# kubeai-project/kubeai

Hardware: AMD Instinct MI355X
Metric: output_tokens_per_s (k6 multi-turn chat) (higher is better)
Workload: dtype fp8; 1 GPU; model=llama-3-8b, global_batch=40, seq_len=8192, parallelism=dp1, prefix_cache=True

## Files before the change

### kubeai_amd/csrc/attention_decode.hip

```cpp
#include <torch/extension.h>

#include <type_traits>

#include "common.h"

namespace {

constexpr int kWaves = 2;
constexpr int kBlockThreads = kWaves * WAVE_SIZE;
constexpr int kBS = 16;
typedef __attribute__((ext_vector_type(2))) __bf16 bf16x2v;
constexpr int kPad = 8;

template <int G, typename CT = ushort, int HD = 128, bool CAP = false>
__launch_bounds__(kBlockThreads) __global__ void paged_decode_kernel(
    ushort* __restrict__ out,
    const ushort* __restrict__ q,
    const CT* __restrict__ k_cache,
    const CT* __restrict__ v_cache,
    const int32_t* __restrict__ block_tables,
    const int32_t* __restrict__ seq_lens,
    const float scale, const float softcap, const int window,
    const int n_kv, const int max_blocks,
    const int64_t q_stride, const int n_splits,
    float* __restrict__ part_o,
    float* __restrict__ part_ml) {
  const int b = blockIdx.x / (n_kv * n_splits);
  const int rem = blockIdx.x % (n_kv * n_splits);
  const int kh = rem / n_splits;
  const int split = rem % n_splits;
  const int n_q = n_kv * G;
  const int wave = threadIdx.x / WAVE_SIZE;
  const int lane = threadIdx.x % WAVE_SIZE;
  const int L = seq_lens[b];
  const int n_blocks = (L + kBS - 1) / kBS;
  const int w0 = (window > 0) ? max(0, L - window) : 0;
  const int blk_base = w0 / kBS;
  const int n_eff = n_blocks - blk_base;
  const int chunk = (n_eff + n_splits - 1) / n_splits;
  const int blk_lo = blk_base + split * chunk;
  const int blk_hi = min(n_blocks, blk_lo + chunk);

  constexpr int PARTS = HD / 32;
  constexpr int TOKP = 64 / PARTS;
  constexpr int EPL = HD / 64;
  __shared__ CT k_lds[kWaves][2][kBS][HD + kPad];
  __shared__ CT v_lds[kWaves][2][kBS][HD + kPad];
  __shared__ float merge_o[kWaves][G][HD];
  __shared__ float merge_ml[kWaves][G][2];

  const int tok_of = lane / PARTS;
  const int part = lane % PARTS;

  uint32_t q_pack[G][16];
#pragma unroll
  for (int g = 0; g < G; ++g) {
    const uint32_t* qp = reinterpret_cast<const uint32_t*>(
        q + (int64_t)b * q_stride + (int64_t)(kh * G + g) * HD + part * 32);
#pragma unroll
    for (int i = 0; i < 16; ++i) q_pack[g][i] = qp[i];
  }

  float m[G], l[G], o[G][EPL];
#pragma unroll
  for (int g = 0; g < G; ++g) {
    m[g] = -INFINITY;
    l[g] = 0.f;
#pragma unroll
    for (int e = 0; e < EPL; ++e) o[g][e] = 0.f;
  }

  const int32_t* bt = block_tables + (int64_t)b * max_blocks;

  using StageVec = std::conditional_t<sizeof(CT) == 2, ushort8, uint64_t>;
  constexpr int NS = (kBS * HD / 8) / WAVE_SIZE;
  StageVec stage_k[NS], stage_v[NS];

  auto issue_loads = [&](int blk_i) {
    const int64_t blk = bt[blk_i];
    const CT* base_k = k_cache + ((blk * n_kv + kh) * kBS) * HD;
    const CT* base_v = v_cache + ((blk * n_kv + kh) * kBS) * HD;
    const StageVec* src_k = reinterpret_cast<const StageVec*>(base_k);
    const StageVec* src_v = reinterpret_cast<const StageVec*>(base_v);
#pragma unroll
    for (int i = 0; i < NS; ++i) {
      stage_k[i] = src_k[lane + i * WAVE_SIZE];
      stage_v[i] = src_v[lane + i * WAVE_SIZE];
    }
  };
  auto write_tile = [&](int buf) {
#pragma unroll
    for (int i = 0; i < NS; ++i) {
      const int vec = lane + i * WAVE_SIZE;
      const int row = vec / (HD / 8);
      const int col = vec % (HD / 8);
      *reinterpret_cast<StageVec*>(&k_lds[wave][buf][row][col * 8]) =
          stage_k[i];
      *reinterpret_cast<StageVec*>(&v_lds[wave][buf][row][col * 8]) =
          stage_v[i];
    }
  };

  const int first = blk_lo + wave;
  int cur = 0;
  if (first < blk_hi) {
    issue_loads(first);
    write_tile(0);
  }

  for (int blk_i = first; blk_i < blk_hi; blk_i += kWaves) {
    const int tile_start = blk_i * kBS;
    const int tile_len = min(kBS, L - tile_start);
    if (blk_i + kWaves < blk_hi) issue_loads(blk_i + kWaves);

#pragma unroll
    for (int tp = 0; tp < kBS; tp += TOKP) {
      const int tok = tp + tok_of;
      float s[G];
#pragma unroll
      for (int g = 0; g < G; ++g) s[g] = 0.f;
      if constexpr (sizeof(CT) == 2) {
        const uint32_t* krow = reinterpret_cast<const uint32_t*>(
            &k_lds[wave][cur][tok][part * 32]);
#pragma unroll
        for (int j = 0; j < 16; ++j) {
          const bf16x2v kk = __builtin_bit_cast(bf16x2v, krow[j]);
#pragma unroll
          for (int g = 0; g < G; ++g)
            s[g] = __builtin_amdgcn_fdot2_f32_bf16(
                kk, __builtin_bit_cast(bf16x2v, q_pack[g][j]), s[g], false);
        }
      } else {
        const uint32_t* krow = reinterpret_cast<const uint32_t*>(
            &k_lds[wave][cur][tok][part * 32]);
#pragma unroll
        for (int j = 0; j < 8; ++j) {
          const uint32_t kk = krow[j];
          const floatx2 k01 = __builtin_amdgcn_cvt_pk_f32_bf8(kk, false);
          const floatx2 k23 = __builtin_amdgcn_cvt_pk_f32_bf8(kk, true);
#pragma unroll
          for (int g = 0; g < G; ++g) {
            const uint32_t qa = q_pack[g][2 * j];
            const uint32_t qb = q_pack[g][2 * j + 1];
            s[g] = fmaf(k01.x, bf16_to_f32((ushort)(qa & 0xffff)), s[g]);
            s[g] = fmaf(k01.y, bf16_to_f32((ushort)(qa >> 16)), s[g]);
            s[g] = fmaf(k23.x, bf16_to_f32((ushort)(qb & 0xffff)), s[g]);
            s[g] = fmaf(k23.y, bf16_to_f32((ushort)(qb >> 16)), s[g]);
          }
        }
      }
      float p[G];
      float rsum[G];
#pragma unroll
      for (int g = 0; g < G; ++g) {
#pragma unroll
        for (int off = 1; off < PARTS; off <<= 1)
          s[g] += __shfl_xor(s[g], off, 64);
        s[g] = (tok < tile_len && tile_start + tok >= w0) ? s[g] * scale
                                                          : -INFINITY;
        if constexpr (CAP) {
          if (s[g] != -INFINITY) s[g] = softcap * tanhf(s[g] / softcap);
        }
        float tmax = s[g];
#pragma unroll
        for (int off = PARTS; off < 64; off <<= 1)
          tmax = fmaxf(tmax, __shfl_xor(tmax, off, 64));
        const float m_new = fmaxf(m[g], tmax);
        if (m_new != m[g]) {
          const float corr = __expf(m[g] - m_new);
          l[g] *= corr;
#pragma unroll
          for (int e = 0; e < EPL; ++e) o[g][e] *= corr;
          m[g] = m_new;
        }
        p[g] = (s[g] == -INFINITY) ? 0.f : __expf(s[g] - m_new);
        rsum[g] = p[g];
#pragma unroll
        for (int off = 1; off < 64; off <<= 1)
          rsum[g] += __shfl_xor(rsum[g], off, 64);
        l[g] += rsum[g] * (1.0f / PARTS);
      }

#pragma unroll
      for (int t = tp; t < tp + TOKP; ++t) {
        if (t >= tile_len) break;
        float vv[EPL];
        if constexpr (sizeof(CT) == 2) {
#pragma unroll
          for (int e = 0; e < EPL; e += 2) {
            const uint32_t vr = *reinterpret_cast<const uint32_t*>(
                &v_lds[wave][cur][t][EPL * lane + e]);
            vv[e] = bf16_to_f32((ushort)(vr & 0xffff));
            vv[e + 1] = bf16_to_f32((ushort)(vr >> 16));
          }
        } else {
#pragma unroll
          for (int e = 0; e < EPL; e += 2) {
            const uint32_t vr = *reinterpret_cast<const ushort*>(
                &v_lds[wave][cur][t][EPL * lane + e]);
            const floatx2 vf = __builtin_amdgcn_cvt_pk_f32_bf8(vr, false);
            vv[e] = vf.x;
            vv[e + 1] = vf.y;
          }
        }
#pragma unroll
        for (int g = 0; g < G; ++g) {
          const float pt = __shfl(p[g], (t - tp) * PARTS, 64);
#pragma unroll
          for (int e = 0; e < EPL; ++e)
            o[g][e] = fmaf(pt, vv[e], o[g][e]);
        }
      }
    }

    if (blk_i + kWaves < blk_hi) write_tile(cur ^ 1);
    cur ^= 1;
  }

#pragma unroll
  for (int g = 0; g < G; ++g) {
#pragma unroll
    for (int e = 0; e < EPL; ++e) merge_o[wave][g][EPL * lane + e] = o[g][e];
    if (lane == 0) {
      merge_ml[wave][g][0] = m[g];
      merge_ml[wave][g][1] = l[g];
    }
  }
  __syncthreads();

  for (int g = wave; g < G; g += kWaves) {
    float m_star = -INFINITY;
#pragma unroll
    for (int w = 0; w < kWaves; ++w) m_star = fmaxf(m_star, merge_ml[w][g][0]);
    float l_star = 0.f, oo[EPL];
#pragma unroll
    for (int e = 0; e < EPL; ++e) oo[e] = 0.f;
    if (m_star != -INFINITY) {
#pragma unroll
      for (int w = 0; w < kWaves; ++w) {
        const float c = __expf(merge_ml[w][g][0] - m_star);
        l_star += merge_ml[w][g][1] * c;
#pragma unroll
        for (int e = 0; e < EPL; ++e)
          oo[e] += merge_o[w][g][EPL * lane + e] * c;
      }
    }
    const int head = kh * G + g;
    if (n_splits == 1) {
      const float inv_l = 1.0f / l_star;
      ushort* oh = out + ((int64_t)b * n_q + head) * HD;
#pragma unroll
      for (int e = 0; e < EPL; e += 2) {
        uint32_t packed =
            ((uint32_t)f32_to_bf16(oo[e + 1] * inv_l) << 16) |
            f32_to_bf16(oo[e] * inv_l);
        *reinterpret_cast<uint32_t*>(&oh[EPL * lane + e]) = packed;
      }
    } else {
      float* po = part_o + (((int64_t)b * n_q + head) * n_splits + split) * HD;
#pragma unroll
      for (int e = 0; e < EPL; ++e) po[EPL * lane + e] = oo[e];
      if (lane == 0) {
        float* pm = part_ml + (((int64_t)b * n_q + head) * n_splits + split) * 2;
        pm[0] = m_star;
        pm[1] = l_star;
      }
    }
  }
}

template <int HD = 128>
__global__ void decode_merge_kernel(
    ushort* __restrict__ out,
    const float* __restrict__ part_o,
    const float* __restrict__ part_ml,
    const int n_q, const int n_splits, const int64_t n_bh) {
  constexpr int EPL = HD / 64;
  const int64_t bh = (int64_t)blockIdx.x * (blockDim.x / WAVE_SIZE) +
                     threadIdx.x / WAVE_SIZE;
  if (bh >= n_bh) return;
  const int lane = threadIdx.x % WAVE_SIZE;
  const float* pml = part_ml + bh * n_splits * 2;
  const float* po = part_o + bh * n_splits * HD;
  float m_star = -INFINITY;
  for (int s = 0; s < n_splits; ++s) m_star = fmaxf(m_star, pml[2 * s]);
  float l_star = 0.f, oo[EPL];
#pragma unroll
  for (int e = 0; e < EPL; ++e) oo[e] = 0.f;
  for (int s = 0; s < n_splits; ++s) {
    const float ms = pml[2 * s];
    if (ms == -INFINITY) continue;
    const float c = __expf(ms - m_star);
    l_star += pml[2 * s + 1] * c;
#pragma unroll
    for (int e = 0; e < EPL; ++e) oo[e] += po[s * HD + EPL * lane + e] * c;
  }
  const float inv_l = 1.0f / l_star;
  ushort* oh = out + bh * HD;
#pragma unroll
  for (int e = 0; e < EPL; e += 2) {
    uint32_t packed = ((uint32_t)f32_to_bf16(oo[e + 1] * inv_l) << 16) |
                      f32_to_bf16(oo[e] * inv_l);
    *reinterpret_cast<uint32_t*>(&oh[EPL * lane + e]) = packed;
  }
}

}

void paged_attention_decode(torch::Tensor out, torch::Tensor q,
                            torch::Tensor k_cache, torch::Tensor v_cache,
                            torch::Tensor block_tables, torch::Tensor seq_lens,
                            double scale, int64_t window, double softcap) {
  TORCH_CHECK(q.stride(2) == 1 && q.stride(1) == q.size(2));
  TORCH_CHECK(out.is_contiguous());
  TORCH_CHECK(k_cache.is_contiguous() && v_cache.is_contiguous());
  TORCH_CHECK(q.scalar_type() == torch::kBFloat16);
  TORCH_CHECK(k_cache.scalar_type() == torch::kBFloat16 ||
              k_cache.scalar_type() == torch::kFloat8_e5m2);
  TORCH_CHECK(block_tables.scalar_type() == torch::kInt32);
  TORCH_CHECK(seq_lens.scalar_type() == torch::kInt32);
  const int B = q.size(0), n_q = q.size(1), hd = q.size(2);
  const int n_kv = k_cache.size(1);
  const int max_blocks = block_tables.size(1);
  TORCH_CHECK(hd == 128 || hd == 256,
              "decode kernel supports head_dim 128 or 256");
  TORCH_CHECK(k_cache.size(2) == kBS, "decode kernel supports block_size=16");
  const int G = n_q / n_kv;
  TORCH_CHECK(n_q % n_kv == 0);
  if (B == 0) return;
  static const int split_target = []() {
    const char* e = getenv("KUBEAI_DECODE_SPLIT_TARGET");
    const int v = e ? atoi(e) : 2048;
    return v > 0 ? v : 2048;
  }();
  static const int min_blocks_per_split = []() {
    const char* e = getenv("KUBEAI_DECODE_MIN_BLOCKS_PER_SPLIT");
    return e ? atoi(e) : 0;
  }();
  int n_splits = 1;
  const int base_wgs = B * n_kv;
  if (base_wgs < split_target) {
    n_splits = std::min<int>(16, (split_target + base_wgs - 1) / base_wgs);
    if (min_blocks_per_split > 0) {
      const int cap = std::max(1, max_blocks / min_blocks_per_split);
      n_splits = std::min(n_splits, cap);
    }
  }
  torch::Tensor part_o, part_ml;
  float *part_o_ptr = nullptr, *part_ml_ptr = nullptr;
  if (n_splits > 1) {
    auto opts =
        torch::TensorOptions().device(q.device()).dtype(torch::kFloat32);
    part_o = torch::empty({B, n_q, n_splits, (int64_t)hd}, opts);
    part_ml = torch::empty({B, n_q, n_splits, 2}, opts);
    part_o_ptr = part_o.data_ptr<float>();
    part_ml_ptr = part_ml.data_ptr<float>();
  }
  dim3 grid(B * n_kv * n_splits), block(kBlockThreads);
  auto stream = c10::hip::getCurrentHIPStream().stream();
  const bool fp8_cache = k_cache.scalar_type() == torch::kFloat8_e5m2;
#define LAUNCH_CT_HD(GG, CT, HDV)                                         \
  do {                                                                    \
    if (softcap > 0.0)                                                    \
      LAUNCH_IMPL(GG, CT, HDV, true);                                     \
    else                                                                  \
      LAUNCH_IMPL(GG, CT, HDV, false);                                    \
  } while (0)
#define LAUNCH_IMPL(GG, CT, HDV, CAPV)                                    \
  hipLaunchKernelGGL((paged_decode_kernel<GG, CT, HDV, CAPV>), grid,      \
                     block, 0,                                            \
                     stream, (ushort*)out.data_ptr(),                     \
                     (const ushort*)q.data_ptr(),                         \
                     (const CT*)k_cache.data_ptr(),                       \
                     (const CT*)v_cache.data_ptr(),                       \
                     block_tables.data_ptr<int32_t>(),                    \
                     seq_lens.data_ptr<int32_t>(), (float)scale,          \
                     (float)softcap, (int)window, n_kv,                   \
                     max_blocks, q.stride(0), n_splits, part_o_ptr,       \
                     part_ml_ptr)
#define LAUNCH(GG)                                                        \
  do {                                                                    \
    if (hd == 256) {                                                      \
              \
      if (fp8_cache) LAUNCH_CT_HD(GG, unsigned char, 256);                \
      else LAUNCH_CT_HD(GG, ushort, 256);                                 \
    } else if (fp8_cache) {                                               \
      LAUNCH_CT_HD(GG, unsigned char, 128);                               \
    } else {                                                              \
      LAUNCH_CT_HD(GG, ushort, 128);                                      \
    }                                                                     \
  } while (0)
  switch (G) {
    case 1: LAUNCH(1); break;
    case 2: LAUNCH(2); break;
    case 4: LAUNCH(4); break;
    case 5: LAUNCH(5); break;
    case 6: LAUNCH(6); break;
    case 8: LAUNCH(8); break;
    default: TORCH_CHECK(false, "unsupported GQA group size ", G);
  }
#undef LAUNCH
#undef LAUNCH_CT_HD
#undef LAUNCH_IMPL
  HIP_CHECK_KERNEL();
  if (n_splits > 1) {
    const int64_t n_bh = (int64_t)B * n_q;
    const int wpb = 4;
    if (hd == 256)
      hipLaunchKernelGGL((decode_merge_kernel<256>),
                         dim3((uint32_t)((n_bh + wpb - 1) / wpb)),
                         dim3(wpb * WAVE_SIZE), 0, stream,
                         (ushort*)out.data_ptr(), part_o_ptr, part_ml_ptr,
                         n_q, n_splits, n_bh);
    else
      hipLaunchKernelGGL((decode_merge_kernel<128>),
                         dim3((uint32_t)((n_bh + wpb - 1) / wpb)),
                         dim3(wpb * WAVE_SIZE), 0, stream,
                         (ushort*)out.data_ptr(), part_o_ptr, part_ml_ptr,
                         n_q, n_splits, n_bh);
    HIP_CHECK_KERNEL();
  }
}
```

### kubeai_amd/csrc/bindings.cpp

```cpp
#include <torch/extension.h>

void rmsnorm(torch::Tensor out, torch::Tensor x, torch::Tensor weight,
             double eps);
void fused_add_rmsnorm(torch::Tensor x, torch::Tensor residual,
                       torch::Tensor weight, double eps);
void rope(torch::Tensor q, torch::Tensor k, torch::Tensor positions,
          torch::Tensor cos_sin);
void reshape_and_cache_fp8(torch::Tensor k, torch::Tensor v,
                           torch::Tensor k_cache, torch::Tensor v_cache,
                           torch::Tensor slot_mapping);
void reshape_and_cache(torch::Tensor k, torch::Tensor v, torch::Tensor k_cache,
                       torch::Tensor v_cache, torch::Tensor slot_mapping);
void paged_attention_decode(torch::Tensor out, torch::Tensor q,
                            torch::Tensor k_cache, torch::Tensor v_cache,
                            torch::Tensor block_tables, torch::Tensor seq_lens,
                            double scale, int64_t window, double softcap);
void paged_attention_prefill(torch::Tensor out, torch::Tensor q,
                             torch::Tensor k_cache, torch::Tensor v_cache,
                             torch::Tensor block_tables,
                             torch::Tensor query_start_loc,
                             torch::Tensor seq_lens, double scale,
                             int64_t window, double softcap);
void silu_and_mul(torch::Tensor out, torch::Tensor x);
void gelu_and_mul(torch::Tensor out, torch::Tensor x);
void skinny_gemm(torch::Tensor y, torch::Tensor x, torch::Tensor w);
void greedy_sample(torch::Tensor out, torch::Tensor logits);
void gumbel_sample(torch::Tensor out, torch::Tensor logits,
                   torch::Tensor temperature, torch::Tensor seeds,
                   int64_t step);
void sgmv(torch::Tensor y, torch::Tensor x, torch::Tensor A, torch::Tensor B,
          torch::Tensor idx, double scale);
void register_chwbl(pybind11::module_& m);
pybind11::bytes xgmi_alloc();
void xgmi_connect(int64_t rank, int64_t world,
                  const std::vector<pybind11::bytes>& handles);
void xgmi_fused_allreduce_add_rmsnorm(torch::Tensor x, torch::Tensor residual,
                                      torch::Tensor weight, double eps);
int64_t xgmi_error_count();
int64_t xgmi_max_elems();
void xgmi_shutdown();
void rmsnorm_fp8(torch::Tensor out, torch::Tensor out_scale, torch::Tensor x,
                 torch::Tensor weight, double eps);
void fused_add_rmsnorm_fp8(torch::Tensor out, torch::Tensor out_scale,
                           torch::Tensor x, torch::Tensor residual,
                           torch::Tensor weight, double eps);
void silu_and_mul_fp8(torch::Tensor out, torch::Tensor out_scale,
                      torch::Tensor x);
void quant_fp8(torch::Tensor out, torch::Tensor out_scale, torch::Tensor x);
void nucleus_stats(torch::Tensor m, torch::Tensor z, torch::Tensor logits,
                   torch::Tensor temps);
void nucleus_accept(torch::Tensor ok, torch::Tensor logits,
                    torch::Tensor cand, torch::Tensor m, torch::Tensor z,
                    torch::Tensor temps, torch::Tensor top_ps,
                    torch::Tensor top_ks);

PYBIND11_MODULE(TORCH_EXTENSION_NAME, m) {
  m.def("rmsnorm", &rmsnorm, "RMSNorm (bf16, fp32 accum)");
  m.def("fused_add_rmsnorm", &fused_add_rmsnorm,
        "in-place residual add + RMSNorm");
  m.def("rope", &rope, "NeoX rotary embedding, in-place q/k");
  m.def("reshape_and_cache", &reshape_and_cache, "paged KV cache write");
  m.def("reshape_and_cache_fp8", &reshape_and_cache_fp8,
        "paged KV cache write, fp8 e5m2 cache");
  m.def("paged_attention_decode", &paged_attention_decode,
        "paged attention, one query token per seq");
  m.def("paged_attention_prefill", &paged_attention_prefill,
        "paged causal flash attention over cached KV");
  m.def("gelu_and_mul", &gelu_and_mul, "GeGLU tanh-gelu(gate)*up");
  m.def("silu_and_mul", &silu_and_mul, "SwiGLU activation");
  m.def("skinny_gemm", &skinny_gemm, "weight-streaming GEMM for M<=64");
  m.def("greedy_sample", &greedy_sample, "argmax sampling");
  m.def("gumbel_sample", &gumbel_sample, "temperature sampling (hash RNG)");
  m.def("rmsnorm_fp8", &rmsnorm_fp8, "rmsnorm with fused fp8 row quant");
  m.def("fused_add_rmsnorm_fp8", &fused_add_rmsnorm_fp8,
        "residual add + rmsnorm with fused fp8 row quant");
  m.def("silu_and_mul_fp8", &silu_and_mul_fp8, "SwiGLU with fused fp8 quant");
  m.def("quant_fp8", &quant_fp8, "bf16 -> fp8 row quant");
  m.def("nucleus_stats", &nucleus_stats, "per-row softmax max + Z");
  m.def("nucleus_accept", &nucleus_accept,
        "nucleus membership of sampled tokens (mass above < p, rank < k)");
  m.def("xgmi_alloc", &xgmi_alloc, "allocate + export the IPC comm buffer");
  m.def("xgmi_connect", &xgmi_connect, "open peer IPC buffers");
  m.def("xgmi_fused_allreduce_add_rmsnorm", &xgmi_fused_allreduce_add_rmsnorm,
        "one-shot xGMI all-reduce fused with residual add + RMSNorm");
  m.def("xgmi_error_count", &xgmi_error_count, "spin-wait timeout count");
  m.def("xgmi_max_elems", &xgmi_max_elems, "one-shot capacity (bf16 elems)");
  m.def("xgmi_shutdown", &xgmi_shutdown, "free/close comm buffers");
  m.def("sgmv", &sgmv, "segmented gather LoRA apply (one adapter segment)");
  register_chwbl(m);
}
```

### kubeai_amd/csrc/common.h

```cpp
#pragma once

#include <hip/hip_runtime.h>
#include <hip/hip_bf16.h>
#include <hip/hip_fp16.h>
#include <hip/hip_fp8.h>
#include <stdint.h>
#include <c10/hip/HIPStream.h>

#define WAVE_SIZE 64
#define DEV_INLINE __device__ __forceinline__

typedef __hip_bfloat16 bf16_t;

typedef ushort __attribute__((ext_vector_type(8))) ushort8;
typedef ushort __attribute__((ext_vector_type(4))) ushort4_t;
typedef float __attribute__((ext_vector_type(4))) float4_t;

DEV_INLINE float bf16_to_f32(ushort u) {
  union {
    uint32_t i;
    float f;
  } c;
  c.i = ((uint32_t)u) << 16;
  return c.f;
}

DEV_INLINE ushort f32_to_bf16(float f) {
  union {
    float f;
    uint32_t i;
  } c;
  c.f = f;
  uint32_t x = c.i;
  uint32_t rb = ((x >> 16) & 1u) + 0x7fffu;
  x += rb;
  return (ushort)(x >> 16);
}


DEV_INLINE float e5m2_to_f32(unsigned char b) {
  const uint32_t s = ((uint32_t)b & 0x80u) << 24;
  uint32_t e = (b >> 2) & 0x1fu;
  uint32_t m = b & 0x3u;
  uint32_t out;
  if (e == 0) {
    if (m == 0) {
      out = s;
    } else {
      int shift = (m & 2u) ? 0 : 1;
      e = 127 - 15 + 1 - 1 - shift;
      m = (m << (shift + 1)) & 0x3u;
      out = s | (e << 23) | (m << 21);
    }
  } else if (e == 0x1fu) {
    out = s | 0x7f800000u | (m << 21);
  } else {
    out = s | ((e - 15u + 127u) << 23) | (m << 21);
  }
  union { uint32_t i; float f; } c;
  c.i = out;
  return c.f;
}

typedef float floatx2 __attribute__((ext_vector_type(2)));

DEV_INLINE ushort8 e5m2x8_to_bf16x8(uint64_t raw) {
  ushort8 out;
#pragma unroll
  for (int j = 0; j < 8; ++j) {
    const ushort h = (ushort)((raw >> (8 * j)) << 8);
    const float f = __half2float(__builtin_bit_cast(__half, h));
    out[j] = (ushort)(__builtin_bit_cast(uint32_t, f) >> 16);
  }
  return out;
}

DEV_INLINE unsigned char f32_to_e5m2(float x) {
  return (unsigned char)__hip_cvt_float_to_fp8(x, __HIP_SATFINITE, __HIP_E5M2);
}


DEV_INLINE float wave_reduce_sum(float v) {
#pragma unroll
  for (int off = 32; off > 0; off >>= 1) v += __shfl_xor(v, off, 64);
  return v;
}

DEV_INLINE float wave_reduce_max(float v) {
#pragma unroll
  for (int off = 32; off > 0; off >>= 1) v = fmaxf(v, __shfl_xor(v, off, 64));
  return v;
}

DEV_INLINE float block_reduce_sum(float v, float* smem) {
  const int wave = threadIdx.x / WAVE_SIZE;
  const int lane = threadIdx.x % WAVE_SIZE;
  const int n_waves = (blockDim.x + WAVE_SIZE - 1) / WAVE_SIZE;
  v = wave_reduce_sum(v);
  if (lane == 0) smem[wave] = v;
  __syncthreads();
  float total = 0.f;
#pragma unroll
  for (int w = 0; w < 16; ++w)
    if (w < n_waves) total += smem[w];
  return total;
}

DEV_INLINE uint64_t splitmix64(uint64_t z) {
  z += 0x9e3779b97f4a7c15ull;
  z = (z ^ (z >> 30)) * 0xbf58476d1ce4e5b9ull;
  z = (z ^ (z >> 27)) * 0x94d049bb133111ebull;
  return z ^ (z >> 31);
}

DEV_INLINE float hash_uniform(uint64_t key, uint64_t idx) {
  uint64_t h = splitmix64(key ^ (idx * 0xd1342543de82ef95ull));
  uint32_t m = (uint32_t)(h >> 40);
  return ((float)m + 1.0f) * (1.0f / 16777216.0f);
}

#define HIP_CHECK_KERNEL()                                    \
  do {                                                        \
    hipError_t e = hipGetLastError();                         \
    if (e != hipSuccess) {                                    \
      TORCH_CHECK(false, "HIP kernel launch failed: ",        \
                  hipGetErrorString(e));                      \
    }                                                         \
  } while (0)
```

### kubeai_amd/csrc/norm.hip

```cpp
#include <torch/extension.h>

#include "common.h"

namespace {

constexpr int kBlock = 256;
constexpr int kMaxVecPerThread = 8;

template <bool kFused>
__global__ void rmsnorm_kernel(
    ushort* __restrict__ out,
    ushort* __restrict__ x,
    ushort* __restrict__ residual,
    const ushort* __restrict__ w,
    const float eps, const int H) {
  const int row = blockIdx.x;
  ushort8* xrow = reinterpret_cast<ushort8*>(x + (int64_t)row * H);
  ushort8* rrow = kFused ? reinterpret_cast<ushort8*>(residual + (int64_t)row * H) : nullptr;
  ushort8* orow = reinterpret_cast<ushort8*>(out + (int64_t)row * H);
  const ushort8* wv = reinterpret_cast<const ushort8*>(w);
  const int nvec = H / 8;

  float vals[kMaxVecPerThread][8];
  float ssum = 0.f;
  int n_iter = 0;
  for (int i = threadIdx.x; i < nvec; i += kBlock, ++n_iter) {
    ushort8 xv = xrow[i];
    ushort8 rin;
    if constexpr (kFused) rin = rrow[i];
#pragma unroll
    for (int j = 0; j < 8; ++j) {
      float f = bf16_to_f32(xv[j]);
      if constexpr (kFused) f += bf16_to_f32(rin[j]);
      vals[n_iter][j] = f;
      ssum += f * f;
    }
    if constexpr (kFused) {
      ushort8 rv;
#pragma unroll
      for (int j = 0; j < 8; ++j) rv[j] = f32_to_bf16(vals[n_iter][j]);
      rrow[i] = rv;
    }
  }

  __shared__ float red[16];
  float total = block_reduce_sum(ssum, red);
  const float inv_rms = rsqrtf(total / (float)H + eps);

  n_iter = 0;
  for (int i = threadIdx.x; i < nvec; i += kBlock, ++n_iter) {
    ushort8 wvv = wv[i];
    ushort8 ov;
#pragma unroll
    for (int j = 0; j < 8; ++j)
      ov[j] = f32_to_bf16(vals[n_iter][j] * inv_rms * bf16_to_f32(wvv[j]));
    orow[i] = ov;
  }
}

}

void rmsnorm(torch::Tensor out, torch::Tensor x, torch::Tensor weight,
             double eps) {
  TORCH_CHECK(x.is_contiguous() && out.is_contiguous());
  TORCH_CHECK(x.scalar_type() == torch::kBFloat16);
  const int H = x.size(-1);
  const int T = x.numel() / H;
  TORCH_CHECK(H % 8 == 0 && H <= kBlock * 8 * kMaxVecPerThread);
  hipLaunchKernelGGL((rmsnorm_kernel<false>), dim3(T), dim3(kBlock), 0,
                     c10::hip::getCurrentHIPStream().stream(),
                     (ushort*)out.data_ptr(), (ushort*)x.data_ptr(), nullptr,
                     (const ushort*)weight.data_ptr(), (float)eps, H);
  HIP_CHECK_KERNEL();
}

void fused_add_rmsnorm(torch::Tensor x, torch::Tensor residual,
                       torch::Tensor weight, double eps) {
  TORCH_CHECK(x.is_contiguous() && residual.is_contiguous());
  TORCH_CHECK(x.scalar_type() == torch::kBFloat16);
  const int H = x.size(-1);
  const int T = x.numel() / H;
  TORCH_CHECK(H % 8 == 0 && H <= kBlock * 8 * kMaxVecPerThread);
  hipLaunchKernelGGL((rmsnorm_kernel<true>), dim3(T), dim3(kBlock), 0,
                     c10::hip::getCurrentHIPStream().stream(),
                     (ushort*)x.data_ptr(), (ushort*)x.data_ptr(),
                     (ushort*)residual.data_ptr(),
                     (const ushort*)weight.data_ptr(), (float)eps, H);
  HIP_CHECK_KERNEL();
}
```

### kubeai_amd/csrc/quant_fp8.hip

```cpp
#include <hip/hip_fp8.h>
#include <torch/extension.h>

#include "common.h"

namespace {

constexpr int kBlock = 256;
constexpr int kMaxVecPerThread = 16;

DEV_INLINE unsigned char f32_to_fp8(float x) {
  return (unsigned char)__hip_cvt_float_to_fp8(x, __HIP_SATFINITE, __HIP_E4M3);
}

DEV_INLINE float block_amax(float v, float* smem) {
  const int wave = threadIdx.x / WAVE_SIZE;
  const int lane = threadIdx.x % WAVE_SIZE;
  const int n_waves = (blockDim.x + WAVE_SIZE - 1) / WAVE_SIZE;
  v = wave_reduce_max(v);
  if (lane == 0) smem[wave] = v;
  __syncthreads();
  float m = 0.f;
#pragma unroll
  for (int w = 0; w < 16; ++w)
    if (w < n_waves) m = fmaxf(m, smem[w]);
  return m;
}

template <bool kFused>
__global__ void rmsnorm_fp8_kernel(
    unsigned char* __restrict__ out,
    float* __restrict__ out_scale,
    ushort* __restrict__ x,
    ushort* __restrict__ residual,
    const ushort* __restrict__ w,
    const float eps, const int H) {
  const int row = blockIdx.x;
  ushort8* xrow = reinterpret_cast<ushort8*>(x + (int64_t)row * H);
  ushort8* rrow =
      kFused ? reinterpret_cast<ushort8*>(residual + (int64_t)row * H) : nullptr;
  const ushort8* wv = reinterpret_cast<const ushort8*>(w);
  const int nvec = H / 8;

  float vals[kMaxVecPerThread][8];
  float ssum = 0.f;
  int n_iter = 0;
  for (int i = threadIdx.x; i < nvec; i += kBlock, ++n_iter) {
    ushort8 xv = xrow[i];
    ushort8 rin;
    if constexpr (kFused) rin = rrow[i];
#pragma unroll
    for (int j = 0; j < 8; ++j) {
      float f = bf16_to_f32(xv[j]);
      if constexpr (kFused) f += bf16_to_f32(rin[j]);
      vals[n_iter][j] = f;
      ssum += f * f;
    }
    if constexpr (kFused) {
      ushort8 rv;
#pragma unroll
      for (int j = 0; j < 8; ++j) rv[j] = f32_to_bf16(vals[n_iter][j]);
      rrow[i] = rv;
    }
  }

  __shared__ float red[16];
  const float total = block_reduce_sum(ssum, red);
  const float inv_rms = rsqrtf(total / (float)H + eps);

  float amax = 0.f;
  n_iter = 0;
  for (int i = threadIdx.x; i < nvec; i += kBlock, ++n_iter) {
    ushort8 wvv = wv[i];
#pragma unroll
    for (int j = 0; j < 8; ++j) {
      vals[n_iter][j] *= inv_rms * bf16_to_f32(wvv[j]);
      amax = fmaxf(amax, fabsf(vals[n_iter][j]));
    }
  }
  __syncthreads();
  const float gmax = fmaxf(block_amax(amax, red), 1e-6f);
  const float scale = gmax / 448.0f;
  if (threadIdx.x == 0) out_scale[row] = scale;
  const float inv_scale = 448.0f / gmax;

  n_iter = 0;
  for (int i = threadIdx.x; i < nvec; i += kBlock, ++n_iter) {
    uchar2 packed[4];
#pragma unroll
    for (int j = 0; j < 4; ++j) {
      packed[j].x = f32_to_fp8(vals[n_iter][2 * j] * inv_scale);
      packed[j].y = f32_to_fp8(vals[n_iter][2 * j + 1] * inv_scale);
    }
    *reinterpret_cast<uint2*>(out + (int64_t)row * H + i * 8) =
        *reinterpret_cast<uint2*>(packed);
  }
}

__global__ void silu_and_mul_fp8_kernel(
    unsigned char* __restrict__ out,
    float* __restrict__ out_scale,
    const ushort* __restrict__ xin,
    const int I) {
  const int row = blockIdx.x;
  const ushort8* gate = reinterpret_cast<const ushort8*>(xin + (int64_t)row * 2 * I);
  const ushort8* up =
      reinterpret_cast<const ushort8*>(xin + (int64_t)row * 2 * I + I);
  const int nvec = I / 8;

  float vals[kMaxVecPerThread][8];
  float amax = 0.f;
  int n_iter = 0;
  for (int i = threadIdx.x; i < nvec; i += kBlock, ++n_iter) {
    ushort8 g = gate[i], u = up[i];
#pragma unroll
    for (int j = 0; j < 8; ++j) {
      const float gf = bf16_to_f32(g[j]);
      const float s = gf / (1.0f + __expf(-gf));
      const float v = s * bf16_to_f32(u[j]);
      vals[n_iter][j] = v;
      amax = fmaxf(amax, fabsf(v));
    }
  }
  __shared__ float red[16];
  const float gmax = fmaxf(block_amax(amax, red), 1e-6f);
  const float scale = gmax / 448.0f;
  if (threadIdx.x == 0) out_scale[row] = scale;
  const float inv_scale = 448.0f / gmax;
  n_iter = 0;
  for (int i = threadIdx.x; i < nvec; i += kBlock, ++n_iter) {
    uchar2 packed[4];
#pragma unroll
    for (int j = 0; j < 4; ++j) {
      packed[j].x = f32_to_fp8(vals[n_iter][2 * j] * inv_scale);
      packed[j].y = f32_to_fp8(vals[n_iter][2 * j + 1] * inv_scale);
    }
    *reinterpret_cast<uint2*>(out + (int64_t)row * I + i * 8) =
        *reinterpret_cast<uint2*>(packed);
  }
}

__global__ void quant_fp8_kernel(unsigned char* __restrict__ out,
                                 float* __restrict__ out_scale,
                                 const ushort* __restrict__ xin, const int H) {
  const int row = blockIdx.x;
  const ushort8* xrow = reinterpret_cast<const ushort8*>(xin + (int64_t)row * H);
  const int nvec = H / 8;
  float vals[kMaxVecPerThread][8];
  float amax = 0.f;
  int n_iter = 0;
  for (int i = threadIdx.x; i < nvec; i += kBlock, ++n_iter) {
    ushort8 xv = xrow[i];
#pragma unroll
    for (int j = 0; j < 8; ++j) {
      const float f = bf16_to_f32(xv[j]);
      vals[n_iter][j] = f;
      amax = fmaxf(amax, fabsf(f));
    }
  }
  __shared__ float red[16];
  const float gmax = fmaxf(block_amax(amax, red), 1e-6f);
  const float scale = gmax / 448.0f;
  if (threadIdx.x == 0) out_scale[row] = scale;
  const float inv_scale = 448.0f / gmax;
  n_iter = 0;
  for (int i = threadIdx.x; i < nvec; i += kBlock, ++n_iter) {
    uchar2 packed[4];
#pragma unroll
    for (int j = 0; j < 4; ++j) {
      packed[j].x = f32_to_fp8(vals[n_iter][2 * j] * inv_scale);
      packed[j].y = f32_to_fp8(vals[n_iter][2 * j + 1] * inv_scale);
    }
    *reinterpret_cast<uint2*>(out + (int64_t)row * H + i * 8) =
        *reinterpret_cast<uint2*>(packed);
  }
}

void check_row_op(const torch::Tensor& x, int max_h) {
  TORCH_CHECK(x.is_contiguous());
  TORCH_CHECK(x.scalar_type() == torch::kBFloat16);
  TORCH_CHECK(x.size(-1) % 8 == 0 && x.size(-1) <= max_h);
}

}

void rmsnorm_fp8(torch::Tensor out, torch::Tensor out_scale, torch::Tensor x,
                 torch::Tensor weight, double eps) {
  check_row_op(x, kBlock * 8 * kMaxVecPerThread);
  const int H = x.size(-1);
  const int T = x.numel() / H;
  hipLaunchKernelGGL((rmsnorm_fp8_kernel<false>), dim3(T), dim3(kBlock), 0,
                     c10::hip::getCurrentHIPStream().stream(),
                     (unsigned char*)out.data_ptr(),
                     out_scale.data_ptr<float>(), (ushort*)x.data_ptr(),
                     nullptr, (const ushort*)weight.data_ptr(), (float)eps, H);
  HIP_CHECK_KERNEL();
}

void fused_add_rmsnorm_fp8(torch::Tensor out, torch::Tensor out_scale,
                           torch::Tensor x, torch::Tensor residual,
                           torch::Tensor weight, double eps) {
  check_row_op(x, kBlock * 8 * kMaxVecPerThread);
  TORCH_CHECK(residual.is_contiguous());
  const int H = x.size(-1);
  const int T = x.numel() / H;
  hipLaunchKernelGGL((rmsnorm_fp8_kernel<true>), dim3(T), dim3(kBlock), 0,
                     c10::hip::getCurrentHIPStream().stream(),
                     (unsigned char*)out.data_ptr(),
                     out_scale.data_ptr<float>(), (ushort*)x.data_ptr(),
                     (ushort*)residual.data_ptr(),
                     (const ushort*)weight.data_ptr(), (float)eps, H);
  HIP_CHECK_KERNEL();
}

void silu_and_mul_fp8(torch::Tensor out, torch::Tensor out_scale,
                      torch::Tensor x) {
  check_row_op(x, 2 * kBlock * 8 * kMaxVecPerThread);
  const int I = x.size(1) / 2;
  TORCH_CHECK(I % 8 == 0 && I <= kBlock * 8 * kMaxVecPerThread);
  const int T = x.size(0);
  if (T == 0) return;
  hipLaunchKernelGGL(silu_and_mul_fp8_kernel, dim3(T), dim3(kBlock), 0,
                     c10::hip::getCurrentHIPStream().stream(),
                     (unsigned char*)out.data_ptr(),
                     out_scale.data_ptr<float>(),
                     (const ushort*)x.data_ptr(), I);
  HIP_CHECK_KERNEL();
}

void quant_fp8(torch::Tensor out, torch::Tensor out_scale, torch::Tensor x) {
  check_row_op(x, kBlock * 8 * kMaxVecPerThread);
  const int H = x.size(-1);
  const int T = x.numel() / H;
  if (T == 0) return;
  hipLaunchKernelGGL(quant_fp8_kernel, dim3(T), dim3(kBlock), 0,
                     c10::hip::getCurrentHIPStream().stream(),
                     (unsigned char*)out.data_ptr(),
                     out_scale.data_ptr<float>(),
                     (const ushort*)x.data_ptr(), H);
  HIP_CHECK_KERNEL();
}
```

### kubeai_amd/csrc/rope.hip

```cpp
#include <torch/extension.h>

#include "common.h"

namespace {

__global__ void rope_kernel(
    ushort* __restrict__ q,
    ushort* __restrict__ k,
    const int32_t* __restrict__ positions,
    const float* __restrict__ cos_sin,
    const int n_q, const int n_kv, const int hd, const int64_t n_tok,
    const int64_t q_stride, const int64_t k_stride) {
  const int n_heads = n_q + n_kv;
  const int64_t flat = (int64_t)blockIdx.x * (blockDim.x / WAVE_SIZE) +
                       threadIdx.x / WAVE_SIZE;
  const int64_t tok = flat / n_heads;
  if (tok >= n_tok) return;
  const int head = (int)(flat % n_heads);
  const int lane = threadIdx.x % WAVE_SIZE;
  const int half = hd / 2;

  const int pos = positions[tok];
  const float* cs = cos_sin + (int64_t)pos * hd;
  ushort* base = (head < n_q)
                     ? q + tok * q_stride + (int64_t)head * hd
                     : k + tok * k_stride + (int64_t)(head - n_q) * hd;

  for (int i = lane; i < half; i += WAVE_SIZE) {
    const float c = cs[i];
    const float s = cs[half + i];
    const float x1 = bf16_to_f32(base[i]);
    const float x2 = bf16_to_f32(base[half + i]);
    base[i] = f32_to_bf16(x1 * c - x2 * s);
    base[half + i] = f32_to_bf16(x2 * c + x1 * s);
  }
}

}

void rope(torch::Tensor q, torch::Tensor k, torch::Tensor positions,
          torch::Tensor cos_sin) {
  TORCH_CHECK(q.stride(2) == 1 && q.stride(1) == q.size(2));
  TORCH_CHECK(k.stride(2) == 1 && k.stride(1) == k.size(2));
  TORCH_CHECK(q.scalar_type() == torch::kBFloat16);
  TORCH_CHECK(positions.scalar_type() == torch::kInt32);
  TORCH_CHECK(cos_sin.scalar_type() == torch::kFloat32);
  const int T = q.size(0);
  const int n_q = q.size(1), n_kv = k.size(1), hd = q.size(2);
  TORCH_CHECK(hd % 2 == 0 && cos_sin.size(1) == hd);
  const int64_t total_waves = (int64_t)T * (n_q + n_kv);
  const int waves_per_block = 4;
  const int64_t blocks = (total_waves + waves_per_block - 1) / waves_per_block;
  hipLaunchKernelGGL(rope_kernel, dim3((uint32_t)blocks),
                     dim3(waves_per_block * WAVE_SIZE), 0,
                     c10::hip::getCurrentHIPStream().stream(), (ushort*)q.data_ptr(),
                     (ushort*)k.data_ptr(),
                     positions.data_ptr<int32_t>(),
                     cos_sin.data_ptr<float>(), n_q, n_kv, hd, (int64_t)T,
                     q.stride(0), k.stride(0));
  HIP_CHECK_KERNEL();
}
```

### kubeai_amd/models/llama.py

```python
from __future__ import annotations

import math

import torch
import torch.nn as nn
import torch.nn.functional as F

from kubeai_amd import ops
from kubeai_amd.engine.batch import ForwardBatch
from .config import ModelArchConfig


class EngineLinear(nn.Linear):

    def forward(self, x: torch.Tensor) -> torch.Tensor:
        y = ops.linear(x, self.weight)
        if self.bias is not None:
            y = y + self.bias
        return y


def _rms_head(x: torch.Tensor, w: torch.Tensor, eps: float) -> torch.Tensor:
    if x.is_cuda and x.dtype == torch.bfloat16:
        flat = x.contiguous().view(-1, x.shape[-1])
        return ops.rmsnorm(flat, w, eps).view(x.shape)
    xf = x.float()
    xf = xf * torch.rsqrt(xf.pow(2).mean(-1, keepdim=True) + eps)
    return (xf * w.float()).to(x.dtype)


class Attention(nn.Module):
    def __init__(self, cfg: ModelArchConfig, layer_idx: int):
        super().__init__()
        self.layer_idx = layer_idx
        self.n_q = cfg.num_attention_heads
        self.n_kv = cfg.num_key_value_heads
        self.hd = cfg.head_dim
        if cfg.global_layer_interval > 0:
            self.is_global = (layer_idx + 1) % cfg.global_layer_interval == 0
            use_win = not self.is_global
        else:
            self.is_global = True
            use_win = (
                cfg.sliding_window_pattern != "even" or layer_idx % 2 == 0
            )
        self.window = (cfg.sliding_window or 0) if use_win else 0
        self.qk_norm = cfg.qk_norm
        if cfg.qk_norm:
            self.q_norm = nn.Parameter(torch.ones(cfg.head_dim))
            self.k_norm = nn.Parameter(torch.ones(cfg.head_dim))
        self.norm_eps = cfg.rms_norm_eps
        self.softcap = cfg.attn_logit_softcap or 0.0
        self.scale = (
            cfg.attention_multiplier
            or 1.0 / math.sqrt(cfg.query_pre_attn_scalar or self.hd)
        )
        q_size = self.n_q * self.hd
        kv_size = self.n_kv * self.hd
        self.qkv_proj = EngineLinear(
            cfg.hidden_size, q_size + 2 * kv_size, bias=cfg.attention_bias
        )
        self.o_proj = EngineLinear(q_size, cfg.hidden_size, bias=False)

    def forward(
        self,
        x: torch.Tensor,
        fb: ForwardBatch,
        kv_cache: tuple[torch.Tensor, torch.Tensor],
        cos_sin: torch.Tensor,
    ) -> torch.Tensor:
        fp8_in = isinstance(x, tuple)
        if fp8_in:
            xq, xs = x
            T = xq.shape[0]
            qkv = self.qkv_proj.forward_quantized(xq, xs)
            lm = None
        else:
            T = x.shape[0]
            qkv = self.qkv_proj(x)
            lm = getattr(self, "_lora_manager", None)
            if lm is not None and lm.active and fb.lora_ids is not None:
                lm.apply(self.layer_idx, "qkv", x, qkv, fb.lora_ids)
        q, k, v = qkv.split(
            [self.n_q * self.hd, self.n_kv * self.hd, self.n_kv * self.hd], dim=-1
        )
        q = q.unflatten(-1, (self.n_q, self.hd))
        k = k.unflatten(-1, (self.n_kv, self.hd))
        v = v.unflatten(-1, (self.n_kv, self.hd))
        if self.qk_norm:
            q = _rms_head(q, self.q_norm, self.norm_eps)
            k = _rms_head(k, self.k_norm, self.norm_eps)
            v = v.contiguous()
        if isinstance(cos_sin, tuple):
            cos_sin = cos_sin[0] if self.is_global else cos_sin[1]
        q, k = ops.rope(q, k, fb.positions, cos_sin)
        k_cache, v_cache = kv_cache
        ops.reshape_and_cache(k, v, k_cache, v_cache, fb.slot_mapping)

        out = torch.empty(
            (T, self.n_q, self.hd), dtype=qkv.dtype, device=qkv.device
        )
        nd = fb.n_decode
        if nd > 0:
            ops.paged_attention_decode(
                q[:nd],
                k_cache,
                v_cache,
                fb.decode_block_tables,
                fb.decode_seq_lens,
                self.scale,
                out=out[:nd],
                window=self.window,
                softcap=self.softcap,
            )
        if fb.n_prefill > 0:
            ops.paged_attention_prefill(
                q[nd:],
                k_cache,
                v_cache,
                fb.prefill_block_tables,
                fb.prefill_query_start_loc,
                fb.prefill_seq_lens,
                self.scale,
                out=out[nd:],
                window=self.window,
                softcap=self.softcap,
            )
        attn_flat = out.view(T, -1)
        if fp8_in:
            a8, ascale = ops.quant_fp8(attn_flat)
            return self.o_proj.forward_quantized(a8, ascale)
        result = self.o_proj(attn_flat)
        if lm is not None and lm.active and fb.lora_ids is not None:
            lm.apply(self.layer_idx, "o", attn_flat, result, fb.lora_ids)
        return result


class MLP(nn.Module):
    def __init__(self, cfg: ModelArchConfig, layer_idx: int | None = None):
        super().__init__()
        self.layer_idx = layer_idx
        self.gate_up_proj = EngineLinear(
            cfg.hidden_size, 2 * cfg.intermediate_size, bias=False
        )
        self.down_proj = EngineLinear(cfg.intermediate_size, cfg.hidden_size, bias=False)
        self.gelu = cfg.hidden_act == "gelu_pytorch_tanh"

    def forward(self, x, fb: ForwardBatch | None = None) -> torch.Tensor:
        if isinstance(x, tuple):
            h = self.gate_up_proj.forward_quantized(*x)
            a8, ascale = ops.silu_and_mul_fp8(h)
            return self.down_proj.forward_quantized(a8, ascale)
        h = self.gate_up_proj(x)
        lm = getattr(self, "_lora_manager", None)
        lora_live = (
            lm is not None and lm.active and fb is not None
            and fb.lora_ids is not None and self.layer_idx is not None
        )
        if lora_live:
            lm.apply(self.layer_idx, "gate_up", x, h, fb.lora_ids)
        a = ops.gelu_and_mul(h) if self.gelu else ops.silu_and_mul(h)
        y = self.down_proj(a)
        if lora_live:
            lm.apply(self.layer_idx, "down", a, y, fb.lora_ids)
        return y


class MoEMLP(nn.Module):

    def __init__(self, cfg: ModelArchConfig):
        super().__init__()
        self.n_experts = cfg.num_local_experts
        self.top_k = cfg.num_experts_per_tok
        self.gate = nn.Linear(cfg.hidden_size, self.n_experts, bias=False)
        self.experts = nn.ModuleList([MLP(cfg) for _ in range(self.n_experts)])

    def forward(self, x: torch.Tensor, fb: ForwardBatch | None = None) -> torch.Tensor:
        T, H = x.shape
        router = F.linear(x.float(), self.gate.weight.float())
        weights, selected = torch.topk(router, self.top_k, dim=-1)
        weights = torch.softmax(weights, dim=-1).to(x.dtype)
        if T <= 256:
            wfull = torch.zeros(T, self.n_experts, dtype=x.dtype,
                                device=x.device)
            wfull.scatter_(1, selected, weights)
            fp8 = hasattr(self.experts[0].gate_up_proj, "forward_quantized")
            if fp8:
                xq, xs = ops.quant_fp8(x)
            out = None
            for e in range(self.n_experts):
                contrib = (
                    self.experts[e]((xq, xs)) if fp8 else self.experts[e](x)
                )
                contrib = contrib * wfull[:, e : e + 1]
                out = contrib if out is None else out + contrib
            return out
        fp8 = hasattr(self.experts[0].gate_up_proj, "forward_quantized")
        if fp8:
            xq, xs = ops.quant_fp8(x)
            xq_bytes = xq.view(torch.uint8)
        out = torch.zeros_like(x)
        for e in range(self.n_experts):
            mask = selected == e
            tok_idx, k_idx = mask.nonzero(as_tuple=True)
            if tok_idx.numel() == 0:
                continue
            if fp8:
                sub = (xq_bytes[tok_idx].view(xq.dtype), xs[tok_idx])
                contrib = self.experts[e](sub)
            else:
                contrib = self.experts[e](x[tok_idx])
            out.index_add_(0, tok_idx, contrib * weights[tok_idx, k_idx, None])
        return out


class DecoderLayer(nn.Module):
    def __init__(self, cfg: ModelArchConfig, layer_idx: int):
        super().__init__()
        self.input_layernorm = nn.Parameter(torch.ones(cfg.hidden_size))
        self.post_attention_layernorm = nn.Parameter(torch.ones(cfg.hidden_size))
        self.self_attn = Attention(cfg, layer_idx)
        self.mlp = (
            MoEMLP(cfg) if cfg.num_local_experts > 0 else MLP(cfg, layer_idx)
        )
        self.eps = cfg.rms_norm_eps
        self.post_norms = cfg.post_norms
        self.res_mult = cfg.residual_multiplier or 1.0
        if cfg.post_norms:
            self.pre_feedforward_layernorm = nn.Parameter(
                torch.ones(cfg.hidden_size)
            )
            self.post_feedforward_layernorm = nn.Parameter(
                torch.ones(cfg.hidden_size)
            )

    def forward(self, x, residual, fb, kv_cache, cos_sin):
        if self.post_norms:
            hidden = x if residual is None else x + residual
            a = self.self_attn(
                ops.rmsnorm(hidden, self.input_layernorm, self.eps),
                fb, kv_cache, cos_sin,
            )
            a = ops.rmsnorm(a, self.post_attention_layernorm, self.eps)
            h2 = hidden + a
            mm = self.mlp(
                ops.rmsnorm(h2, self.pre_feedforward_layernorm, self.eps), fb
            )
            mm = ops.rmsnorm(mm, self.post_feedforward_layernorm, self.eps)
            return mm, h2
        if (
            getattr(self, "_fp8_fused", False)
            and x.is_cuda
            and fb.lora_ids is None
        ):
            if residual is None:
                residual = x
                xq, xs = ops.rmsnorm_fp8(x, self.input_layernorm, self.eps)
            else:
                xq, xs = ops.fused_add_rmsnorm_fp8(
                    x, residual, self.input_layernorm, self.eps
                )
            x = self.self_attn((xq, xs), fb, kv_cache, cos_sin)
            if isinstance(self.mlp, MoEMLP):
                x, residual = ops.fused_add_rmsnorm(
                    x, residual, self.post_attention_layernorm, self.eps
                )
                x = self.mlp(x)
            else:
                xq, xs = ops.fused_add_rmsnorm_fp8(
                    x, residual, self.post_attention_layernorm, self.eps
                )
                x = self.mlp((xq, xs))
            return x, residual
        if residual is None:
            residual = x
            x = ops.rmsnorm(x, self.input_layernorm, self.eps)
        else:
            x, residual = ops.fused_add_rmsnorm(
                x, residual, self.input_layernorm, self.eps
            )
        x = self.self_attn(x, fb, kv_cache, cos_sin)
        if self.res_mult != 1.0:
            x = x * self.res_mult
        x, residual = ops.fused_add_rmsnorm(
            x, residual, self.post_attention_layernorm, self.eps
        )
        x = self.mlp(x, fb)
        if self.res_mult != 1.0:
            x = x * self.res_mult
        return x, residual


class LlamaForCausalLM(nn.Module):

    def __init__(self, cfg: ModelArchConfig, device=None, dtype=torch.bfloat16):
        super().__init__()
        self.cfg = cfg
        prev_dtype = torch.get_default_dtype()
        torch.set_default_dtype(dtype)
        try:
            with torch.device(device if device is not None else "cpu"):
                self.embed_tokens = nn.Embedding(cfg.vocab_size, cfg.hidden_size)
                self.layers = nn.ModuleList(
                    [DecoderLayer(cfg, i) for i in range(cfg.num_hidden_layers)]
                )
                self.norm = nn.Parameter(torch.ones(cfg.hidden_size))
                if cfg.tie_word_embeddings:
                    self.lm_head = None
                else:
                    self.lm_head = EngineLinear(
                        cfg.hidden_size, cfg.vocab_size, bias=False
                    )
        finally:
            torch.set_default_dtype(prev_dtype)
        from kubeai_amd.ops import ref as ops_ref

        self.register_buffer(
            "cos_sin",
            ops_ref.make_cos_sin_cache(
                cfg.head_dim, cfg.max_position_embeddings, cfg.rope_theta,
                rope_scaling=cfg.rope_scaling,
            ).to(device=device),
            persistent=False,
        )
        if cfg.rope_local_base_freq:
            self.register_buffer(
                "cos_sin_local",
                ops_ref.make_cos_sin_cache(
                    cfg.head_dim, cfg.max_position_embeddings,
                    cfg.rope_local_base_freq,
                ).to(device=device),
                persistent=False,
            )
        else:
            self.cos_sin_local = None

    @torch.inference_mode()
    def forward(self, fb: ForwardBatch) -> torch.Tensor:
        cs = (
            (self.cos_sin, self.cos_sin_local)
            if self.cos_sin_local is not None
            else self.cos_sin
        )
        x = self.embed_tokens(fb.input_ids.long())
        if self.cfg.scale_embeddings:
            x = x * torch.tensor(
                self.cfg.hidden_size ** 0.5, dtype=x.dtype
            )
        elif self.cfg.embedding_multiplier:
            x = x * self.cfg.embedding_multiplier
        if fb.mm_embeds is not None:
            x = x.index_copy(0, fb.mm_idx, fb.mm_embeds.to(x.dtype))
        residual = None
        for i, layer in enumerate(self.layers):
            x, residual = layer(x, residual, fb, self.kv_caches[i], cs)
        x, _ = ops.fused_add_rmsnorm(x, residual, self.norm, self.cfg.rms_norm_eps)
        return x

    @torch.inference_mode()
    def compute_logits(self, hidden: torch.Tensor) -> torch.Tensor:
        if self.lm_head is None:
            logits = F.linear(hidden, self.embed_tokens.weight).float()
        else:
            logits = self.lm_head(hidden).float()
        if self.cfg.logits_scaling:
            logits = logits / self.cfg.logits_scaling
        cap = self.cfg.final_logit_softcap
        if cap > 0:
            logits = cap * torch.tanh(logits / cap)
        return logits

    def bind_kv_caches(self, kv_caches: list[tuple[torch.Tensor, torch.Tensor]]):
        self.kv_caches = kv_caches
```

### kubeai_amd/ops/__init__.py

```python
from __future__ import annotations

import torch

from . import ref

_C = None
_C_IMPORT_ERROR: Exception | None = None
try:
    from kubeai_amd import _C
except Exception as e:
    _C_IMPORT_ERROR = e


def have_hip_ext() -> bool:
    return _C is not None


def _require_ext() -> None:
    if _C is None:
        raise RuntimeError(
            "kubeai_amd HIP extension (kubeai_amd._C) is not built but a GPU "
            "tensor reached the ops layer. Build it with "
            "`python setup.py build_ext --inplace` (PYTORCH_ROCM_ARCH=gfx950). "
            f"Original import error: {_C_IMPORT_ERROR!r}"
        )


def rmsnorm(x: torch.Tensor, weight: torch.Tensor, eps: float) -> torch.Tensor:
    if x.is_cuda:
        _require_ext()
        out = torch.empty_like(x)
        _C.rmsnorm(out, x, weight, eps)
        return out
    return ref.rmsnorm(x, weight, eps)


def fused_add_rmsnorm(x, residual, weight, eps: float):
    if x.is_cuda:
        _require_ext()
        _C.fused_add_rmsnorm(x, residual, weight, eps)
        return x, residual
    return ref.fused_add_rmsnorm(x, residual, weight, eps)


def rope(q, k, positions, cos_sin):
    if q.is_cuda:
        _require_ext()
        _C.rope(q, k, positions, cos_sin)
        return q, k
    return ref.rope(q, k, positions, cos_sin)


def reshape_and_cache(k, v, k_cache, v_cache, slot_mapping) -> None:
    if k.is_cuda:
        _require_ext()
        if k_cache.dtype == torch.float8_e5m2:
            _C.reshape_and_cache_fp8(k, v, k_cache, v_cache, slot_mapping)
        else:
            _C.reshape_and_cache(k, v, k_cache, v_cache, slot_mapping)
        return
    ref.reshape_and_cache(k, v, k_cache, v_cache, slot_mapping)


def paged_attention_decode(
    q, k_cache, v_cache, block_tables, seq_lens, scale: float, out=None,
    window: int = 0, softcap: float = 0.0,
):
    if q.is_cuda:
        _require_ext()
        if out is None:
            out = torch.empty(q.shape, dtype=q.dtype, device=q.device)
        _C.paged_attention_decode(
            out, q, k_cache, v_cache, block_tables, seq_lens, scale, window,
            softcap
        )
        return out
    res = ref.paged_attention_decode(
        q, k_cache, v_cache, block_tables, seq_lens, scale, window=window,
        softcap=softcap,
    )
    if out is not None:
        out.copy_(res)
        return out
    return res


def paged_attention_prefill(
    q, k_cache, v_cache, block_tables, query_start_loc, seq_lens, scale: float,
    out=None, window: int = 0, softcap: float = 0.0,
):
    if q.is_cuda:
        _require_ext()
        if out is None:
            out = torch.empty(q.shape, dtype=q.dtype, device=q.device)
        _C.paged_attention_prefill(
            out, q, k_cache, v_cache, block_tables, query_start_loc, seq_lens,
            scale, window, softcap
        )
        return out
    res = ref.paged_attention_prefill(
        q, k_cache, v_cache, block_tables, query_start_loc, seq_lens, scale,
        window=window, softcap=softcap,
    )
    if out is not None:
        out.copy_(res)
        return out
    return res


def silu_and_mul(x):
    if x.is_cuda:
        _require_ext()
        T, two_i = x.shape
        out = torch.empty((T, two_i // 2), dtype=x.dtype, device=x.device)
        _C.silu_and_mul(out, x)
        return out
    return ref.silu_and_mul(x)


def gelu_and_mul(x):
    if x.is_cuda:
        _require_ext()
        T, two_i = x.shape
        out = torch.empty((T, two_i // 2), dtype=x.dtype, device=x.device)
        _C.gelu_and_mul(out, x)
        return out
    return ref.gelu_and_mul(x)


import os

_USE_SKINNY = os.environ.get("KUBEAI_SKINNY_GEMM", "0") == "1"


def linear(x, weight):
    if (
        _USE_SKINNY
        and x.is_cuda
        and x.dtype == torch.bfloat16
        and x.dim() == 2
        and 1 <= x.shape[0] <= 64
        and weight.shape[1] % 64 == 0
        and weight.shape[0] % 64 == 0
        and x.is_contiguous()
        and weight.is_contiguous()
    ):
        _require_ext()
        y = torch.empty(
            (x.shape[0], weight.shape[0]), dtype=x.dtype, device=x.device
        )
        _C.skinny_gemm(y, x, weight)
        return y
    return torch.nn.functional.linear(x, weight)


def rmsnorm_fp8(x, weight, eps: float):
    _require_ext()
    out = torch.empty(x.shape, dtype=torch.float8_e4m3fn, device=x.device)
    scale = torch.empty(x.shape[0], dtype=torch.float32, device=x.device)
    _C.rmsnorm_fp8(out, scale, x, weight, eps)
    return out, scale


def fused_add_rmsnorm_fp8(x, residual, weight, eps: float):
    _require_ext()
    out = torch.empty(x.shape, dtype=torch.float8_e4m3fn, device=x.device)
    scale = torch.empty(x.shape[0], dtype=torch.float32, device=x.device)
    _C.fused_add_rmsnorm_fp8(out, scale, x, residual, weight, eps)
    return out, scale


def silu_and_mul_fp8(x):
    if not x.is_cuda:
        return ref.quant_fp8(ref.silu_and_mul(x))
    _require_ext()
    T, two_i = x.shape
    out = torch.empty((T, two_i // 2), dtype=torch.float8_e4m3fn, device=x.device)
    scale = torch.empty(T, dtype=torch.float32, device=x.device)
    _C.silu_and_mul_fp8(out, scale, x)
    return out, scale


def quant_fp8(x):
    if not x.is_cuda:
        return ref.quant_fp8(x)
    _require_ext()
    out = torch.empty(x.shape, dtype=torch.float8_e4m3fn, device=x.device)
    scale = torch.empty(x.shape[0], dtype=torch.float32, device=x.device)
    _C.quant_fp8(out, scale, x)
    return out, scale


def greedy_sample(logits):
    if logits.is_cuda:
        _require_ext()
        out = torch.empty(logits.shape[0], dtype=torch.int64, device=logits.device)
        _C.greedy_sample(out, logits)
        return out
    return ref.greedy_sample(logits)


def gumbel_sample(logits, temperature, seeds, step: int):
    if logits.is_cuda:
        _require_ext()
        out = torch.empty(logits.shape[0], dtype=torch.int64, device=logits.device)
        _C.gumbel_sample(out, logits, temperature, seeds, step)
        return out
    return ref.gumbel_sample(logits, temperature, seeds, step)


def nucleus_stats(logits, temps):
    if logits.is_cuda:
        _require_ext()
        S = logits.shape[0]
        m = torch.empty(S, dtype=torch.float32, device=logits.device)
        z = torch.empty_like(m)
        _C.nucleus_stats(m, z, logits, temps)
        return m, z
    t = temps.clamp_min(1e-6).unsqueeze(1)
    m = logits.max(dim=-1).values
    z = torch.exp((logits - m.unsqueeze(1)) / t).sum(-1)
    return m, z


def nucleus_accept(logits, cand, m, z, temps, top_ps, top_ks):
    if logits.is_cuda:
        _require_ext()
        ok = torch.empty(logits.shape[0], dtype=torch.uint8,
                         device=logits.device)
        _C.nucleus_accept(ok, logits, cand, m, z, temps, top_ps, top_ks)
        return ok
    t = temps.clamp_min(1e-6).unsqueeze(1)
    lt = logits.gather(1, cand.view(-1, 1))
    above = logits > lt
    mass = (torch.exp((logits - m.unsqueeze(1)) / t) * above).sum(-1) / z
    cnt = above.sum(-1)
    ok = (mass < top_ps) & ((top_ks <= 0) | (cnt < top_ks)) | (temps <= 0)
    return ok.to(torch.uint8)
```

### kubeai_amd/parallel/tp.py

```python
from __future__ import annotations

import math
import os

import torch
import torch.distributed as dist
import torch.nn as nn
import torch.nn.functional as F

from kubeai_amd import ops
from kubeai_amd.engine.batch import ForwardBatch
from kubeai_amd.models.config import ModelArchConfig
from kubeai_amd.models.llama import EngineLinear


class TPGroup:
    def __init__(self, group=None):
        self.group = group
        self.rank = dist.get_rank(group)
        self.world = dist.get_world_size(group)
        self._xgmi = None
        self._xgmi_tried = False

    def all_reduce(self, t: torch.Tensor) -> torch.Tensor:
        if self.world > 1:
            dist.all_reduce(t, group=self.group)
        return t

    def _xgmi_comm(self, t: torch.Tensor):
        if not self._xgmi_tried:
            self._xgmi_tried = True
            if (
                self.world > 1
                and t.is_cuda
                and os.environ.get("KUBEAI_XGMI_ALLREDUCE", "1") == "1"
            ):
                try:
                    from .comm import XgmiAllReduce

                    self._xgmi = XgmiAllReduce(self.group, t.device)
                except Exception:
                    import traceback

                    traceback.print_exc()
                    self._xgmi = None
        return self._xgmi

    def allreduce_add_rmsnorm(self, x, residual, weight, eps):
        if self.world > 1:
            comm = self._xgmi_comm(x)
            if comm is not None and comm.fits(x):
                return comm.fused_allreduce_add_rmsnorm(x, residual, weight, eps)
            dist.all_reduce(x, group=self.group)
        return ops.fused_add_rmsnorm(x, residual, weight, eps)

    def allreduce_add_rmsnorm_fp8(self, x, residual, weight, eps):
        if self.world > 1:
            comm = self._xgmi_comm(x)
            if comm is not None and comm.fits(x):
                x, residual = comm.fused_allreduce_add_rmsnorm(
                    x, residual, weight, eps
                )
                return ops.quant_fp8(x), residual
            dist.all_reduce(x, group=self.group)
        xq_xs = ops.fused_add_rmsnorm_fp8(x, residual, weight, eps)
        return xq_xs, residual


def _shard_rows(full: torch.Tensor, tp: TPGroup) -> torch.Tensor:
    n = full.shape[0] // tp.world
    return full[tp.rank * n : (tp.rank + 1) * n].clone()


def _shard_cols(full: torch.Tensor, tp: TPGroup) -> torch.Tensor:
    n = full.shape[1] // tp.world
    return full[:, tp.rank * n : (tp.rank + 1) * n].clone()


def _full_weight(shape, gen) -> torch.Tensor:
    return torch.randn(shape, generator=gen) / math.sqrt(shape[1])


class TPAttention(nn.Module):
    def __init__(self, cfg: ModelArchConfig, layer_idx: int, tp: TPGroup):
        super().__init__()
        self.tp = tp
        self.layer_idx = layer_idx
        assert cfg.num_attention_heads % tp.world == 0, "q heads % tp != 0"
        assert cfg.num_key_value_heads % tp.world == 0, "kv heads % tp != 0"
        self.n_q = cfg.num_attention_heads // tp.world
        self.n_kv = cfg.num_key_value_heads // tp.world
        self.hd = cfg.head_dim
        self.window = cfg.sliding_window or 0
        self.scale = 1.0 / math.sqrt(self.hd)
        H = cfg.hidden_size
        self.qkv_proj = EngineLinear(H, (self.n_q + 2 * self.n_kv) * self.hd, bias=False)
        self.o_proj = EngineLinear(self.n_q * self.hd, H, bias=False)

    def shard_from_full(self, full_qkv: torch.Tensor, full_o: torch.Tensor,
                        cfg: ModelArchConfig) -> None:
        tp = self.tp
        nq, nkv, hd = cfg.num_attention_heads, cfg.num_key_value_heads, cfg.head_dim
        q_w = full_qkv[: nq * hd]
        k_w = full_qkv[nq * hd : (nq + nkv) * hd]
        v_w = full_qkv[(nq + nkv) * hd :]
        qs = _shard_rows(q_w.view(nq, hd, -1), tp).reshape(self.n_q * hd, -1)
        ks = _shard_rows(k_w.view(nkv, hd, -1), tp).reshape(self.n_kv * hd, -1)
        vs = _shard_rows(v_w.view(nkv, hd, -1), tp).reshape(self.n_kv * hd, -1)
        self.qkv_proj.weight.data.copy_(torch.cat([qs, ks, vs], dim=0))
        self.o_proj.weight.data.copy_(
            full_o[:, tp.rank * self.n_q * hd : (tp.rank + 1) * self.n_q * hd].clone()
        )

    def forward(self, x, fb: ForwardBatch, kv_cache, cos_sin):
        fp8_in = isinstance(x, tuple)
        if fp8_in:
            xq, xs = x
            T = xq.shape[0]
            qkv = self.qkv_proj.forward_quantized(xq, xs)
        else:
            T = x.shape[0]
            qkv = self.qkv_proj(x)
        q, k, v = qkv.split(
            [self.n_q * self.hd, self.n_kv * self.hd, self.n_kv * self.hd], dim=-1
        )
        q = q.unflatten(-1, (self.n_q, self.hd))
        k = k.unflatten(-1, (self.n_kv, self.hd))
        v = v.unflatten(-1, (self.n_kv, self.hd))
        q, k = ops.rope(q, k, fb.positions, cos_sin)
        k_cache, v_cache = kv_cache
        ops.reshape_and_cache(k, v, k_cache, v_cache, fb.slot_mapping)
        out = torch.empty(
            (T, self.n_q, self.hd), dtype=qkv.dtype, device=qkv.device
        )
        nd = fb.n_decode
        if nd > 0:
            ops.paged_attention_decode(
                q[:nd], k_cache, v_cache,
                fb.decode_block_tables, fb.decode_seq_lens, self.scale,
                out=out[:nd], window=getattr(self, "window", 0),
            )
        if fb.n_prefill > 0:
            ops.paged_attention_prefill(
                q[nd:], k_cache, v_cache,
                fb.prefill_block_tables, fb.prefill_query_start_loc,
                fb.prefill_seq_lens, self.scale,
                out=out[nd:], window=getattr(self, "window", 0),
            )
        attn_flat = out.view(T, -1)
        if fp8_in:
            a8, ascale = ops.quant_fp8(attn_flat)
            return self.o_proj.forward_quantized(a8, ascale)
        return self.o_proj(attn_flat)


class TPMLP(nn.Module):
    def __init__(self, cfg: ModelArchConfig, tp: TPGroup):
        super().__init__()
        self.tp = tp
        assert cfg.intermediate_size % tp.world == 0
        self.i_local = cfg.intermediate_size // tp.world
        self.gate_up_proj = EngineLinear(cfg.hidden_size, 2 * self.i_local, bias=False)
        self.down_proj = EngineLinear(self.i_local, cfg.hidden_size, bias=False)

    def shard_from_full(self, full_gate_up: torch.Tensor, full_down: torch.Tensor,
                        cfg: ModelArchConfig) -> None:
        I = cfg.intermediate_size
        r, w = self.tp.rank, self.tp.world
        gate = full_gate_up[:I][r * self.i_local : (r + 1) * self.i_local]
        up = full_gate_up[I:][r * self.i_local : (r + 1) * self.i_local]
        self.gate_up_proj.weight.data.copy_(torch.cat([gate, up], dim=0))
        self.down_proj.weight.data.copy_(
            full_down[:, r * self.i_local : (r + 1) * self.i_local]
        )

    def forward(self, x):
        if isinstance(x, tuple):
            h = self.gate_up_proj.forward_quantized(*x)
            a8, ascale = ops.silu_and_mul_fp8(h)
            return self.down_proj.forward_quantized(a8, ascale)
        act = ops.silu_and_mul(self.gate_up_proj(x))
        return self.down_proj(act)


class TPDecoderLayer(nn.Module):
    def __init__(self, cfg: ModelArchConfig, layer_idx: int, tp: TPGroup):
        super().__init__()
        self.input_layernorm = nn.Parameter(torch.ones(cfg.hidden_size))
        self.post_attention_layernorm = nn.Parameter(torch.ones(cfg.hidden_size))
        self.self_attn = TPAttention(cfg, layer_idx, tp)
        self.mlp = TPMLP(cfg, tp)
        self.eps = cfg.rms_norm_eps

    def forward(self, x, residual, fb, kv_cache, cos_sin):
        tp = self.self_attn.tp
        fp8 = (
            getattr(self, "_fp8_fused", False)
            and fb.lora_ids is None
            and (x.is_cuda if not isinstance(x, tuple) else True)
        )
        if residual is None:
            residual = x
            if fp8:
                xin = ops.rmsnorm_fp8(x, self.input_layernorm, self.eps)
            else:
                xin = ops.rmsnorm(x, self.input_layernorm, self.eps)
        elif fp8:
            xin, residual = tp.allreduce_add_rmsnorm_fp8(
                x, residual, self.input_layernorm, self.eps
            )
        else:
            xin, residual = tp.allreduce_add_rmsnorm(
                x, residual, self.input_layernorm, self.eps
            )
        x = self.self_attn(xin, fb, kv_cache, cos_sin)
        if fp8:
            xmid, residual = tp.allreduce_add_rmsnorm_fp8(
                x, residual, self.post_attention_layernorm, self.eps
            )
        else:
            xmid, residual = tp.allreduce_add_rmsnorm(
                x, residual, self.post_attention_layernorm, self.eps
            )
        x = self.mlp(xmid)
        return x, residual


class TPLlamaForCausalLM(nn.Module):

    def __init__(self, cfg: ModelArchConfig, tp: TPGroup, device=None,
                 dtype=torch.bfloat16, seed: int = 0):
        super().__init__()
        self.cfg = cfg
        self.tp = tp
        self.n_kv_local = cfg.num_key_value_heads // tp.world
        gen = torch.Generator().manual_seed(seed)
        H = cfg.hidden_size
        self.embed_tokens = nn.Embedding(cfg.vocab_size, H)
        emb_full = torch.randn(cfg.vocab_size, H, generator=gen)
        self.embed_tokens.weight.data.copy_(emb_full)
        self.layers = nn.ModuleList(
            [TPDecoderLayer(cfg, i, tp) for i in range(cfg.num_hidden_layers)]
        )
        nq, nkv, hd = cfg.num_attention_heads, cfg.num_key_value_heads, cfg.head_dim
        for layer in self.layers:
            full_qkv = _full_weight(((nq + 2 * nkv) * hd, H), gen)
            full_o = _full_weight((H, nq * hd), gen)
            layer.self_attn.shard_from_full(full_qkv, full_o, cfg)
            full_gate_up = _full_weight((2 * cfg.intermediate_size, H), gen)
            full_down = _full_weight((H, cfg.intermediate_size), gen)
            layer.mlp.shard_from_full(full_gate_up, full_down, cfg)
        self.norm = nn.Parameter(torch.ones(H))
        if cfg.tie_word_embeddings:
            self.lm_head = None
        else:
            self.lm_head = EngineLinear(H, cfg.vocab_size, bias=False)
            self.lm_head.weight.data.copy_(_full_weight((cfg.vocab_size, H), gen))
        self.to(device=device, dtype=dtype)
        from kubeai_amd.ops import ref as ops_ref

        self.register_buffer(
            "cos_sin",
            ops_ref.make_cos_sin_cache(
                cfg.head_dim, cfg.max_position_embeddings, cfg.rope_theta,
                rope_scaling=cfg.rope_scaling,
            ).to(device=device),
            persistent=False,
        )

    @torch.inference_mode()
    def forward(self, fb: ForwardBatch) -> torch.Tensor:
        x = self.embed_tokens(fb.input_ids.long())
        if fb.mm_embeds is not None:
            x = x.index_copy(0, fb.mm_idx, fb.mm_embeds.to(x.dtype))
        residual = None
        for i, layer in enumerate(self.layers):
            x, residual = layer(x, residual, fb, self.kv_caches[i], self.cos_sin)
        x, _ = self.tp.allreduce_add_rmsnorm(
            x, residual, self.norm, self.cfg.rms_norm_eps
        )
        return x

    @torch.inference_mode()
    def compute_logits(self, hidden: torch.Tensor) -> torch.Tensor:
        if self.lm_head is None:
            return F.linear(hidden, self.embed_tokens.weight).float()
        return self.lm_head(hidden).float()

    def bind_kv_caches(self, kv_caches):
        self.kv_caches = kv_caches
```

Baseline: 6558 tok/s.

## Fuse rope with KV cache write and decode merge with fp8 quantization

Adds a rope_and_cache kernel that rotates q/k and writes k/v into the paged cache in one launch, replacing separate rope and reshape_and_cache calls. Adds a decode merge kernel that, for pure-decode fp8 batches, merges split partials and emits the per-row e4m3 quantized output and scale directly, skipping the separate quant_fp8 pass before o_proj. Also templates rmsnorm on a compile-time iteration count with weight preloading. These cut kernel launches and extra memory round trips per layer in decode. The fused merge uses one block per sequence, which may underuse the GPU at small batch.

Result: faster. 7190 tok/s (median of 6 runs) (+9.6%).

```diff
diff --git a/kubeai_amd/csrc/attention_decode.hip b/kubeai_amd/csrc/attention_decode.hip
--- a/kubeai_amd/csrc/attention_decode.hip
+++ b/kubeai_amd/csrc/attention_decode.hip
@@ -269,6 +269,32 @@
   }
 }
 
+template <int N, int HD>
+DEV_INLINE void merge_partials(const float* __restrict__ po,
+                               const float* __restrict__ pml,
+                               const int n_splits, uint32_t (&packed)[N / 2]) {
+  typedef float __attribute__((ext_vector_type(N))) vecN;
+  float m_star = -INFINITY;
+  for (int s = 0; s < n_splits; ++s) m_star = fmaxf(m_star, pml[2 * s]);
+  float l_star = 0.f, oo[N];
+#pragma unroll
+  for (int e = 0; e < N; ++e) oo[e] = 0.f;
+  for (int s = 0; s < n_splits; ++s) {
+    const float ms = pml[2 * s];
+    if (ms == -INFINITY) continue;
+    const float c = __expf(ms - m_star);
+    l_star += pml[2 * s + 1] * c;
+    const vecN pv = *reinterpret_cast<const vecN*>(po + s * HD);
+#pragma unroll
+    for (int e = 0; e < N; ++e) oo[e] += pv[e] * c;
+  }
+  const float inv_l = 1.0f / l_star;
+#pragma unroll
+  for (int e = 0; e < N; e += 2)
+    packed[e / 2] = ((uint32_t)f32_to_bf16(oo[e + 1] * inv_l) << 16) |
+                    f32_to_bf16(oo[e] * inv_l);
+}
+
 template <int HD = 128>
 __global__ void decode_merge_kernel(
     ushort* __restrict__ out,
@@ -280,37 +306,87 @@
                      threadIdx.x / WAVE_SIZE;
   if (bh >= n_bh) return;
   const int lane = threadIdx.x % WAVE_SIZE;
-  const float* pml = part_ml + bh * n_splits * 2;
-  const float* po = part_o + bh * n_splits * HD;
-  float m_star = -INFINITY;
-  for (int s = 0; s < n_splits; ++s) m_star = fmaxf(m_star, pml[2 * s]);
-  float l_star = 0.f, oo[EPL];
-#pragma unroll
-  for (int e = 0; e < EPL; ++e) oo[e] = 0.f;
-  for (int s = 0; s < n_splits; ++s) {
-    const float ms = pml[2 * s];
-    if (ms == -INFINITY) continue;
-    const float c = __expf(ms - m_star);
-    l_star += pml[2 * s + 1] * c;
-#pragma unroll
-    for (int e = 0; e < EPL; ++e) oo[e] += po[s * HD + EPL * lane + e] * c;
-  }
-  const float inv_l = 1.0f / l_star;
+  uint32_t packed[EPL / 2];
+  merge_partials<EPL, HD>(part_o + bh * n_splits * HD + EPL * lane,
+                          part_ml + bh * n_splits * 2, n_splits, packed);
   ushort* oh = out + bh * HD;
 #pragma unroll
-  for (int e = 0; e < EPL; e += 2) {
-    uint32_t packed = ((uint32_t)f32_to_bf16(oo[e + 1] * inv_l) << 16) |
-                      f32_to_bf16(oo[e] * inv_l);
-    *reinterpret_cast<uint32_t*>(&oh[EPL * lane + e]) = packed;
-  }
-}
-
-}
-
-void paged_attention_decode(torch::Tensor out, torch::Tensor q,
-                            torch::Tensor k_cache, torch::Tensor v_cache,
-                            torch::Tensor block_tables, torch::Tensor seq_lens,
-                            double scale, int64_t window, double softcap) {
+  for (int e = 0; e < EPL; e += 2)
+    *reinterpret_cast<uint32_t*>(&oh[EPL * lane + e]) = packed[e / 2];
+}
+
+constexpr int kMergeVec = 4;
+constexpr int kMergeMaxThreads = 1024;
+constexpr int kMergeMaxPasses = 2;
+constexpr int kMergeRowMax = kMergeMaxThreads * kMergeVec * kMergeMaxPasses;
+
+template <int HD, int kPasses>
+__launch_bounds__(kMergeMaxThreads) __global__ void decode_merge_fp8_kernel(
+    ushort* __restrict__ out,
+    unsigned char* __restrict__ out_fp8,
+    float* __restrict__ out_scale,
+    const float* __restrict__ part_o,
+    const float* __restrict__ part_ml,
+    const int n_q, const int n_splits) {
+  __shared__ float red[16];
+  const int b = blockIdx.x;
+  const int row_len = n_q * HD;
+  const int nvec = row_len / kMergeVec;
+  ushort* orow = out + (int64_t)b * row_len;
+
+  uint32_t packed[kPasses][kMergeVec / 2];
+  float amax = 0.f;
+#pragma unroll
+  for (int it = 0; it < kPasses; ++it) {
+    const int i = threadIdx.x + it * blockDim.x;
+    if (i < nvec) {
+      const int h = (i * kMergeVec) / HD;
+      const int col = (i * kMergeVec) % HD;
+      const int64_t bh = (int64_t)b * n_q + h;
+      merge_partials<kMergeVec, HD>(part_o + bh * n_splits * HD + col,
+                                    part_ml + bh * n_splits * 2, n_splits,
+                                    packed[it]);
+      *reinterpret_cast<uint2*>(orow + i * kMergeVec) =
+          make_uint2(packed[it][0], packed[it][1]);
+#pragma unroll
+      for (int e = 0; e < kMergeVec / 2; ++e) {
+        const uint32_t pk = packed[it][e];
+        amax = fmaxf(amax, fabsf(bf16_to_f32((ushort)(pk & 0xffff))));
+        amax = fmaxf(amax, fabsf(bf16_to_f32((ushort)(pk >> 16))));
+      }
+    }
+  }
+  const float gmax = fmaxf(block_amax(amax, red), 1e-6f);
+  const float scale = gmax / 448.0f;
+  if (threadIdx.x == 0) out_scale[b] = scale;
+  const float inv_scale = 448.0f / gmax;
+  unsigned char* frow = out_fp8 + (int64_t)b * row_len;
+#pragma unroll
+  for (int it = 0; it < kPasses; ++it) {
+    const int i = threadIdx.x + it * blockDim.x;
+    if (i < nvec) {
+      uchar4 q4;
+      const uint32_t p0 = packed[it][0], p1 = packed[it][1];
+      q4.x = f32_to_fp8(bf16_to_f32((ushort)(p0 & 0xffff)) * inv_scale);
+      q4.y = f32_to_fp8(bf16_to_f32((ushort)(p0 >> 16)) * inv_scale);
+      q4.z = f32_to_fp8(bf16_to_f32((ushort)(p1 & 0xffff)) * inv_scale);
+      q4.w = f32_to_fp8(bf16_to_f32((ushort)(p1 >> 16)) * inv_scale);
+      *reinterpret_cast<uchar4*>(frow + i * kMergeVec) = q4;
+    }
+  }
+}
+
+}
+
+void quant_fp8(torch::Tensor out, torch::Tensor out_scale, torch::Tensor x);
+
+namespace {
+
+void decode_impl(torch::Tensor out, torch::Tensor q, torch::Tensor k_cache,
+                 torch::Tensor v_cache, torch::Tensor block_tables,
+                 torch::Tensor seq_lens, double scale, int64_t window,
+                 double softcap, torch::Tensor* out_fp8,
+                 torch::Tensor* out_scale) {
   TORCH_CHECK(q.stride(2) == 1 && q.stride(1) == q.size(2));
   TORCH_CHECK(out.is_contiguous());
   TORCH_CHECK(k_cache.is_contiguous() && v_cache.is_contiguous());
@@ -403,6 +479,31 @@
 #undef LAUNCH_CT_HD
 #undef LAUNCH_IMPL
   HIP_CHECK_KERNEL();
+  const bool want_fp8 = out_fp8 != nullptr;
+  const bool fuse_fp8 =
+      want_fp8 && n_splits > 1 && (int64_t)n_q * hd <= kMergeRowMax;
+  if (fuse_fp8) {
+    const int nvec = n_q * hd / kMergeVec;
+    const int threads = std::min(
+        kMergeMaxThreads, (nvec + WAVE_SIZE - 1) / WAVE_SIZE * WAVE_SIZE);
+    const int passes = (nvec + threads - 1) / threads;
+#define LAUNCH_MERGE_FP8(HDV, PASSES)                                       \
+  hipLaunchKernelGGL((decode_merge_fp8_kernel<HDV, PASSES>), dim3(B),       \
+                     dim3(threads), 0, stream, (ushort*)out.data_ptr(),     \
+                     (unsigned char*)out_fp8->data_ptr(),                   \
+                     out_scale->data_ptr<float>(), part_o_ptr, part_ml_ptr, \
+                     n_q, n_splits)
+    if (hd == 256) {
+      if (passes == 1) LAUNCH_MERGE_FP8(256, 1);
+      else LAUNCH_MERGE_FP8(256, 2);
+    } else {
+      if (passes == 1) LAUNCH_MERGE_FP8(128, 1);
+      else LAUNCH_MERGE_FP8(128, 2);
+    }
+#undef LAUNCH_MERGE_FP8
+    HIP_CHECK_KERNEL();
+    return;
+  }
   if (n_splits > 1) {
     const int64_t n_bh = (int64_t)B * n_q;
     const int wpb = 4;
@@ -420,4 +521,30 @@
                          n_q, n_splits, n_bh);
     HIP_CHECK_KERNEL();
   }
-}
+  if (want_fp8) quant_fp8(*out_fp8, *out_scale, out.view({B, -1}));
+}
+
+}
+
+void paged_attention_decode(torch::Tensor out, torch::Tensor q,
+                            torch::Tensor k_cache, torch::Tensor v_cache,
+                            torch::Tensor block_tables, torch::Tensor seq_lens,
+                            double scale, int64_t window, double softcap) {
+  decode_impl(out, q, k_cache, v_cache, block_tables, seq_lens, scale, window,
+              softcap, nullptr, nullptr);
+}
+
+void paged_attention_decode_fp8(torch::Tensor out, torch::Tensor out_fp8,
+                                torch::Tensor out_scale, torch::Tensor q,
+                                torch::Tensor k_cache, torch::Tensor v_cache,
+                                torch::Tensor block_tables,
+                                torch::Tensor seq_lens, double scale,
+                                int64_t window, double softcap) {
+  TORCH_CHECK(out_fp8.is_contiguous() && out_scale.is_contiguous());
+  TORCH_CHECK(out_fp8.scalar_type() == torch::kFloat8_e4m3fn);
+  TORCH_CHECK(out_scale.scalar_type() == torch::kFloat32);
+  TORCH_CHECK(out_fp8.numel() == out.numel() &&
+              out_scale.numel() == out.size(0));
+  decode_impl(out, q, k_cache, v_cache, block_tables, seq_lens, scale, window,
+              softcap, &out_fp8, &out_scale);
+}
diff --git a/kubeai_amd/csrc/bindings.cpp b/kubeai_amd/csrc/bindings.cpp
--- a/kubeai_amd/csrc/bindings.cpp
+++ b/kubeai_amd/csrc/bindings.cpp
@@ -6,6 +6,10 @@
                        torch::Tensor weight, double eps);
 void rope(torch::Tensor q, torch::Tensor k, torch::Tensor positions,
           torch::Tensor cos_sin);
+void rope_and_cache(torch::Tensor q, torch::Tensor k, torch::Tensor v,
+                    torch::Tensor positions, torch::Tensor cos_sin,
+                    torch::Tensor k_cache, torch::Tensor v_cache,
+                    torch::Tensor slot_mapping);
 void reshape_and_cache_fp8(torch::Tensor k, torch::Tensor v,
                            torch::Tensor k_cache, torch::Tensor v_cache,
                            torch::Tensor slot_mapping);
@@ -15,6 +19,12 @@
                             torch::Tensor k_cache, torch::Tensor v_cache,
                             torch::Tensor block_tables, torch::Tensor seq_lens,
                             double scale, int64_t window, double softcap);
+void paged_attention_decode_fp8(torch::Tensor out, torch::Tensor out_fp8,
+                                torch::Tensor out_scale, torch::Tensor q,
+                                torch::Tensor k_cache, torch::Tensor v_cache,
+                                torch::Tensor block_tables,
+                                torch::Tensor seq_lens, double scale,
+                                int64_t window, double softcap);
 void paged_attention_prefill(torch::Tensor out, torch::Tensor q,
                              torch::Tensor k_cache, torch::Tensor v_cache,
                              torch::Tensor block_tables,
@@ -59,11 +69,15 @@
   m.def("fused_add_rmsnorm", &fused_add_rmsnorm,
         "in-place residual add + RMSNorm");
   m.def("rope", &rope, "NeoX rotary embedding, in-place q/k");
+  m.def("rope_and_cache", &rope_and_cache,
+        "rotary embedding (in-place q/k) fused with the paged KV cache write");
   m.def("reshape_and_cache", &reshape_and_cache, "paged KV cache write");
   m.def("reshape_and_cache_fp8", &reshape_and_cache_fp8,
         "paged KV cache write, fp8 e5m2 cache");
   m.def("paged_attention_decode", &paged_attention_decode,
         "paged attention, one query token per seq");
+  m.def("paged_attention_decode_fp8", &paged_attention_decode_fp8,
+        "paged decode attention that also emits the e4m3 row quant of out");
   m.def("paged_attention_prefill", &paged_attention_prefill,
         "paged causal flash attention over cached KV");
   m.def("gelu_and_mul", &gelu_and_mul, "GeGLU tanh-gelu(gate)*up");
diff --git a/kubeai_amd/csrc/common.h b/kubeai_amd/csrc/common.h
--- a/kubeai_amd/csrc/common.h
+++ b/kubeai_amd/csrc/common.h
@@ -79,6 +79,12 @@
   return (unsigned char)__hip_cvt_float_to_fp8(x, __HIP_SATFINITE, __HIP_E5M2);
 }
 
+DEV_INLINE void rope_rotate_pair(const float x1, const float x2, const float c,
+                                 const float s, ushort& o1, ushort& o2) {
+  o1 = f32_to_bf16(x1 * c - x2 * s);
+  o2 = f32_to_bf16(x2 * c + x1 * s);
+}
+
 
 DEV_INLINE float wave_reduce_sum(float v) {
 #pragma unroll
@@ -106,6 +112,34 @@
   return total;
 }
 
+DEV_INLINE float block_amax(float v, float* smem) {
+  const int wave = threadIdx.x / WAVE_SIZE;
+  const int lane = threadIdx.x % WAVE_SIZE;
+  const int n_waves = (blockDim.x + WAVE_SIZE - 1) / WAVE_SIZE;
+  v = wave_reduce_max(v);
+  if (lane == 0) smem[wave] = v;
+  __syncthreads();
+  float m = 0.f;
+#pragma unroll
+  for (int w = 0; w < 16; ++w)
+    if (w < n_waves) m = fmaxf(m, smem[w]);
+  return m;
+}
+
+DEV_INLINE unsigned char f32_to_fp8(float x) {
+  return (unsigned char)__hip_cvt_float_to_fp8(x, __HIP_SATFINITE, __HIP_E4M3);
+}
+
+DEV_INLINE uint2 quant8_fp8(const float (&f)[8], const float inv_scale) {
+  uchar2 packed[4];
+#pragma unroll
+  for (int j = 0; j < 4; ++j) {
+    packed[j].x = f32_to_fp8(f[2 * j] * inv_scale);
+    packed[j].y = f32_to_fp8(f[2 * j + 1] * inv_scale);
+  }
+  return *reinterpret_cast<uint2*>(packed);
+}
+
 DEV_INLINE uint64_t splitmix64(uint64_t z) {
   z += 0x9e3779b97f4a7c15ull;
   z = (z ^ (z >> 30)) * 0xbf58476d1ce4e5b9ull;
diff --git a/kubeai_amd/csrc/norm.hip b/kubeai_amd/csrc/norm.hip
--- a/kubeai_amd/csrc/norm.hip
+++ b/kubeai_amd/csrc/norm.hip
@@ -5,10 +5,10 @@
 namespace {
 
 constexpr int kBlock = 256;
-constexpr int kMaxVecPerThread = 8;
+constexpr int kMaxIters = 8;
 
-template <bool kFused>
-__global__ void rmsnorm_kernel(
+template <bool kFused, int kIters>
+__launch_bounds__(kBlock) __global__ void rmsnorm_kernel(
     ushort* __restrict__ out,
     ushort* __restrict__ x,
     ushort* __restrict__ residual,
@@ -21,42 +21,62 @@
   const ushort8* wv = reinterpret_cast<const ushort8*>(w);
   const int nvec = H / 8;
 
-  float vals[kMaxVecPerThread][8];
+  float vals[kIters][8];
   float ssum = 0.f;
-  int n_iter = 0;
-  for (int i = threadIdx.x; i < nvec; i += kBlock, ++n_iter) {
-    ushort8 xv = xrow[i];
-    ushort8 rin;
-    if constexpr (kFused) rin = rrow[i];
 #pragma unroll
-    for (int j = 0; j < 8; ++j) {
-      float f = bf16_to_f32(xv[j]);
-      if constexpr (kFused) f += bf16_to_f32(rin[j]);
-      vals[n_iter][j] = f;
-      ssum += f * f;
+  for (int it = 0; it < kIters; ++it) {
+    const int i = threadIdx.x + it * kBlock;
+    if (i < nvec) {
+      ushort8 xv = xrow[i];
+      ushort8 rin;
+      if constexpr (kFused) rin = rrow[i];
+#pragma unroll
+      for (int j = 0; j < 8; ++j) {
+        float f = bf16_to_f32(xv[j]);
+        if constexpr (kFused) f += bf16_to_f32(rin[j]);
+        vals[it][j] = f;
+        ssum += f * f;
+      }
+      if constexpr (kFused) {
+        ushort8 rv;
+#pragma unroll
+        for (int j = 0; j < 8; ++j) rv[j] = f32_to_bf16(vals[it][j]);
+        rrow[i] = rv;
+      }
     }
-    if constexpr (kFused) {
-      ushort8 rv;
+  }
+  ushort8 wreg[kIters];
 #pragma unroll
-      for (int j = 0; j < 8; ++j) rv[j] = f32_to_bf16(vals[n_iter][j]);
-      rrow[i] = rv;
-    }
+  for (int it = 0; it < kIters; ++it) {
+    const int i = threadIdx.x + it * kBlock;
+    if (i < nvec) wreg[it] = wv[i];
   }
 
   __shared__ float red[16];
   float total = block_reduce_sum(ssum, red);
   const float inv_rms = rsqrtf(total / (float)H + eps);
 
-  n_iter = 0;
-  for (int i = threadIdx.x; i < nvec; i += kBlock, ++n_iter) {
-    ushort8 wvv = wv[i];
-    ushort8 ov;
 #pragma unroll
-    for (int j = 0; j < 8; ++j)
-      ov[j] = f32_to_bf16(vals[n_iter][j] * inv_rms * bf16_to_f32(wvv[j]));
-    orow[i] = ov;
+  for (int it = 0; it < kIters; ++it) {
+    const int i = threadIdx.x + it * kBlock;
+    if (i < nvec) {
+      ushort8 ov;
+#pragma unroll
+      for (int j = 0; j < 8; ++j)
+        ov[j] = f32_to_bf16(vals[it][j] * inv_rms * bf16_to_f32(wreg[it][j]));
+      orow[i] = ov;
+    }
   }
 }
+
+#define NORM_DISPATCH(nvec, LAUNCH)                   \
+  do {                                                \
+    const int n_it_ = ((nvec) + kBlock - 1) / kBlock; \
+    if (n_it_ <= 1) { LAUNCH(1); }                    \
+    else if (n_it_ <= 2) { LAUNCH(2); }               \
+    else if (n_it_ <= 4) { LAUNCH(4); }               \
+    else { LAUNCH(8); }                               \
+  } while (0)
 
 }
 
@@ -66,11 +86,14 @@
   TORCH_CHECK(x.scalar_type() == torch::kBFloat16);
   const int H = x.size(-1);
   const int T = x.numel() / H;
-  TORCH_CHECK(H % 8 == 0 && H <= kBlock * 8 * kMaxVecPerThread);
-  hipLaunchKernelGGL((rmsnorm_kernel<false>), dim3(T), dim3(kBlock), 0,
-                     c10::hip::getCurrentHIPStream().stream(),
-                     (ushort*)out.data_ptr(), (ushort*)x.data_ptr(), nullptr,
-                     (const ushort*)weight.data_ptr(), (float)eps, H);
+  TORCH_CHECK(H % 8 == 0 && H <= kBlock * 8 * kMaxIters);
+#define LAUNCH_ROW(ITERS)                                                     \
+  hipLaunchKernelGGL((rmsnorm_kernel<false, ITERS>), dim3(T), dim3(kBlock),   \
+                     0, c10::hip::getCurrentHIPStream().stream(),             \
+                     (ushort*)out.data_ptr(), (ushort*)x.data_ptr(), nullptr, \
+                     (const ushort*)weight.data_ptr(), (float)eps, H)
+  NORM_DISPATCH(H / 8, LAUNCH_ROW);
+#undef LAUNCH_ROW
   HIP_CHECK_KERNEL();
 }
 
@@ -80,11 +103,14 @@
   TORCH_CHECK(x.scalar_type() == torch::kBFloat16);
   const int H = x.size(-1);
   const int T = x.numel() / H;
-  TORCH_CHECK(H % 8 == 0 && H <= kBlock * 8 * kMaxVecPerThread);
-  hipLaunchKernelGGL((rmsnorm_kernel<true>), dim3(T), dim3(kBlock), 0,
-                     c10::hip::getCurrentHIPStream().stream(),
-                     (ushort*)x.data_ptr(), (ushort*)x.data_ptr(),
-                     (ushort*)residual.data_ptr(),
-                     (const ushort*)weight.data_ptr(), (float)eps, H);
+  TORCH_CHECK(H % 8 == 0 && H <= kBlock * 8 * kMaxIters);
+#define LAUNCH_ROW(ITERS)                                                   \
+  hipLaunchKernelGGL((rmsnorm_kernel<true, ITERS>), dim3(T), dim3(kBlock),  \
+                     0, c10::hip::getCurrentHIPStream().stream(),           \
+                     (ushort*)x.data_ptr(), (ushort*)x.data_ptr(),          \
+                     (ushort*)residual.data_ptr(),                          \
+                     (const ushort*)weight.data_ptr(), (float)eps, H)
+  NORM_DISPATCH(H / 8, LAUNCH_ROW);
+#undef LAUNCH_ROW
   HIP_CHECK_KERNEL();
 }
diff --git a/kubeai_amd/csrc/quant_fp8.hip b/kubeai_amd/csrc/quant_fp8.hip
--- a/kubeai_amd/csrc/quant_fp8.hip
+++ b/kubeai_amd/csrc/quant_fp8.hip
@@ -6,28 +6,24 @@
 namespace {
 
 constexpr int kBlock = 256;
-constexpr int kMaxVecPerThread = 16;
-
-DEV_INLINE unsigned char f32_to_fp8(float x) {
-  return (unsigned char)__hip_cvt_float_to_fp8(x, __HIP_SATFINITE, __HIP_E4M3);
-}
-
-DEV_INLINE float block_amax(float v, float* smem) {
-  const int wave = threadIdx.x / WAVE_SIZE;
-  const int lane = threadIdx.x % WAVE_SIZE;
-  const int n_waves = (blockDim.x + WAVE_SIZE - 1) / WAVE_SIZE;
-  v = wave_reduce_max(v);
-  if (lane == 0) smem[wave] = v;
-  __syncthreads();
-  float m = 0.f;
-#pragma unroll
-  for (int w = 0; w < 16; ++w)
-    if (w < n_waves) m = fmaxf(m, smem[w]);
-  return m;
-}
-
-template <bool kFused>
-__global__ void rmsnorm_fp8_kernel(
+constexpr int kBlockWide = 512;
+constexpr int kMaxIters = 8;
+constexpr int kMaxH = kBlockWide * 8 * kMaxIters;
+
+template <int kThreads, int kIters>
+DEV_INLINE void store_row_fp8(unsigned char* __restrict__ orow,
+                              const float (&vals)[kIters][8],
+                              const float inv_scale, const int nvec) {
+#pragma unroll
+  for (int it = 0; it < kIters; ++it) {
+    const int i = threadIdx.x + it * kThreads;
+    if (i < nvec)
+      *reinterpret_cast<uint2*>(orow + i * 8) = quant8_fp8(vals[it], inv_scale);
+  }
+}
+
+template <bool kFused, int kThreads, int kIters>
+__launch_bounds__(kThreads) __global__ void rmsnorm_fp8_kernel(
     unsigned char* __restrict__ out,
     float* __restrict__ out_scale,
     ushort* __restrict__ x,
@@ -41,26 +37,35 @@
   const ushort8* wv = reinterpret_cast<const ushort8*>(w);
   const int nvec = H / 8;
 
-  float vals[kMaxVecPerThread][8];
+  float vals[kIters][8];
   float ssum = 0.f;
-  int n_iter = 0;
-  for (int i = threadIdx.x; i < nvec; i += kBlock, ++n_iter) {
-    ushort8 xv = xrow[i];
-    ushort8 rin;
-    if constexpr (kFused) rin = rrow[i];
-#pragma unroll
-    for (int j = 0; j < 8; ++j) {
-      float f = bf16_to_f32(xv[j]);
-      if constexpr (kFused) f += bf16_to_f32(rin[j]);
-      vals[n_iter][j] = f;
-      ssum += f * f;
-    }
-    if constexpr (kFused) {
-      ushort8 rv;
-#pragma unroll
-      for (int j = 0; j < 8; ++j) rv[j] = f32_to_bf16(vals[n_iter][j]);
-      rrow[i] = rv;
-    }
+#pragma unroll
+  for (int it = 0; it < kIters; ++it) {
+    const int i = threadIdx.x + it * kThreads;
+    if (i < nvec) {
+      ushort8 xv = xrow[i];
+      ushort8 rin;
+      if constexpr (kFused) rin = rrow[i];
+#pragma unroll
+      for (int j = 0; j < 8; ++j) {
+        float f = bf16_to_f32(xv[j]);
+        if constexpr (kFused) f += bf16_to_f32(rin[j]);
+        vals[it][j] = f;
+        ssum += f * f;
+      }
+      if constexpr (kFused) {
+        ushort8 rv;
+#pragma unroll
+        for (int j = 0; j < 8; ++j) rv[j] = f32_to_bf16(vals[it][j]);
+        rrow[i] = rv;
+      }
+    }
+  }
+  ushort8 wreg[kIters];
+#pragma unroll
+  for (int it = 0; it < kIters; ++it) {
+    const int i = threadIdx.x + it * kThreads;
+    if (i < nvec) wreg[it] = wv[i];
   }
 
   __shared__ float red[16];
@@ -68,13 +73,15 @@
   const float inv_rms = rsqrtf(total / (float)H + eps);
 
   float amax = 0.f;
-  n_iter = 0;
-  for (int i = threadIdx.x; i < nvec; i += kBlock, ++n_iter) {
-    ushort8 wvv = wv[i];
-#pragma unroll
-    for (int j = 0; j < 8; ++j) {
-      vals[n_iter][j] *= inv_rms * bf16_to_f32(wvv[j]);
-      amax = fmaxf(amax, fabsf(vals[n_iter][j]));
+#pragma unroll
+  for (int it = 0; it < kIters; ++it) {
+    const int i = threadIdx.x + it * kThreads;
+    if (i < nvec) {
+#pragma unroll
+      for (int j = 0; j < 8; ++j) {
+        vals[it][j] *= inv_rms * bf16_to_f32(wreg[it][j]);
+        amax = fmaxf(amax, fabsf(vals[it][j]));
+      }
     }
   }
   __syncthreads();
@@ -82,21 +89,11 @@
   const float scale = gmax / 448.0f;
   if (threadIdx.x == 0) out_scale[row] = scale;
   const float inv_scale = 448.0f / gmax;
-
-  n_iter = 0;
-  for (int i = threadIdx.x; i < nvec; i += kBlock, ++n_iter) {
-    uchar2 packed[4];
-#pragma unroll
-    for (int j = 0; j < 4; ++j) {
-      packed[j].x = f32_to_fp8(vals[n_iter][2 * j] * inv_scale);
-      packed[j].y = f32_to_fp8(vals[n_iter][2 * j + 1] * inv_scale);
-    }
-    *reinterpret_cast<uint2*>(out + (int64_t)row * H + i * 8) =
-        *reinterpret_cast<uint2*>(packed);
-  }
-}
-
-__global__ void silu_and_mul_fp8_kernel(
+  store_row_fp8<kThreads, kIters>(out + (int64_t)row * H, vals, inv_scale, nvec);
+}
+
+template <int kThreads, int kIters>
+__launch_bounds__(kThreads) __global__ void silu_and_mul_fp8_kernel(
     unsigned char* __restrict__ out,
     float* __restrict__ out_scale,
     const ushort* __restrict__ xin,
@@ -107,18 +104,21 @@
       reinterpret_cast<const ushort8*>(xin + (int64_t)row * 2 * I + I);
   const int nvec = I / 8;
 
-  float vals[kMaxVecPerThread][8];
+  float vals[kIters][8];
   float amax = 0.f;
-  int n_iter = 0;
-  for (int i = threadIdx.x; i < nvec; i += kBlock, ++n_iter) {
-    ushort8 g = gate[i], u = up[i];
-#pragma unroll
-    for (int j = 0; j < 8; ++j) {
-      const float gf = bf16_to_f32(g[j]);
-      const float s = gf / (1.0f + __expf(-gf));
-      const float v = s * bf16_to_f32(u[j]);
-      vals[n_iter][j] = v;
-      amax = fmaxf(amax, fabsf(v));
+#pragma unroll
+  for (int it = 0; it < kIters; ++it) {
+    const int i = threadIdx.x + it * kThreads;
+    if (i < nvec) {
+      ushort8 g = gate[i], u = up[i];
+#pragma unroll
+      for (int j = 0; j < 8; ++j) {
+        const float gf = bf16_to_f32(g[j]);
+        const float s = gf / (1.0f + __expf(-gf));
+        const float v = s * bf16_to_f32(u[j]);
+        vals[it][j] = v;
+        amax = fmaxf(amax, fabsf(v));
+      }
     }
   }
   __shared__ float red[16];
@@ -126,35 +126,29 @@
   const float scale = gmax / 448.0f;
   if (threadIdx.x == 0) out_scale[row] = scale;
   const float inv_scale = 448.0f / gmax;
-  n_iter = 0;
-  for (int i = threadIdx.x; i < nvec; i += kBlock, ++n_iter) {
-    uchar2 packed[4];
-#pragma unroll
-    for (int j = 0; j < 4; ++j) {
-      packed[j].x = f32_to_fp8(vals[n_iter][2 * j] * inv_scale);
-      packed[j].y = f32_to_fp8(vals[n_iter][2 * j + 1] * inv_scale);
-    }
-    *reinterpret_cast<uint2*>(out + (int64_t)row * I + i * 8) =
-        *reinterpret_cast<uint2*>(packed);
-  }
-}
-
-__global__ void quant_fp8_kernel(unsigned char* __restrict__ out,
-                                 float* __restrict__ out_scale,
-                                 const ushort* __restrict__ xin, const int H) {
+  store_row_fp8<kThreads, kIters>(out + (int64_t)row * I, vals, inv_scale, nvec);
+}
+
+template <int kThreads, int kIters>
+__launch_bounds__(kThreads) __global__ void quant_fp8_kernel(
+    unsigned char* __restrict__ out, float* __restrict__ out_scale,
+    const ushort* __restrict__ xin, const int H) {
   const int row = blockIdx.x;
   const ushort8* xrow = reinterpret_cast<const ushort8*>(xin + (int64_t)row * H);
   const int nvec = H / 8;
-  float vals[kMaxVecPerThread][8];
+  float vals[kIters][8];
   float amax = 0.f;
-  int n_iter = 0;
-  for (int i = threadIdx.x; i < nvec; i += kBlock, ++n_iter) {
-    ushort8 xv = xrow[i];
-#pragma unroll
-    for (int j = 0; j < 8; ++j) {
-      const float f = bf16_to_f32(xv[j]);
-      vals[n_iter][j] = f;
-      amax = fmaxf(amax, fabsf(f));
+#pragma unroll
+  for (int it = 0; it < kIters; ++it) {
+    const int i = threadIdx.x + it * kThreads;
+    if (i < nvec) {
+      ushort8 xv = xrow[i];
+#pragma unroll
+      for (int j = 0; j < 8; ++j) {
+        const float f = bf16_to_f32(xv[j]);
+        vals[it][j] = f;
+        amax = fmaxf(amax, fabsf(f));
+      }
     }
   }
   __shared__ float red[16];
@@ -162,17 +156,7 @@
   const float scale = gmax / 448.0f;
   if (threadIdx.x == 0) out_scale[row] = scale;
   const float inv_scale = 448.0f / gmax;
-  n_iter = 0;
-  for (int i = threadIdx.x; i < nvec; i += kBlock, ++n_iter) {
-    uchar2 packed[4];
-#pragma unroll
-    for (int j = 0; j < 4; ++j) {
-      packed[j].x = f32_to_fp8(vals[n_iter][2 * j] * inv_scale);
-      packed[j].y = f32_to_fp8(vals[n_iter][2 * j + 1] * inv_scale);
-    }
-    *reinterpret_cast<uint2*>(out + (int64_t)row * H + i * 8) =
-        *reinterpret_cast<uint2*>(packed);
-  }
+  store_row_fp8<kThreads, kIters>(out + (int64_t)row * H, vals, inv_scale, nvec);
 }
 
 void check_row_op(const torch::Tensor& x, int max_h) {
@@ -181,61 +165,104 @@
   TORCH_CHECK(x.size(-1) % 8 == 0 && x.size(-1) <= max_h);
 }
 
+#define ROW_DISPATCH_ITERS(THREADS, nvec, LAUNCH)              \
+  do {                                                         \
+    const int n_it_ = ((nvec) + (THREADS)-1) / (THREADS);      \
+    if (n_it_ <= 1) { LAUNCH(THREADS, 1); }                    \
+    else if (n_it_ <= 2) { LAUNCH(THREADS, 2); }               \
+    else if (n_it_ <= 4) { LAUNCH(THREADS, 4); }               \
+    else { LAUNCH(THREADS, 8); }                               \
+  } while (0)
+
+#define ROW_DISPATCH_NORM(nvec, LAUNCH)                        \
+  do {                                                         \
+    if ((nvec) <= kBlock * kMaxIters)                          \
+      ROW_DISPATCH_ITERS(kBlock, nvec, LAUNCH);                \
+    else                                                       \
+      LAUNCH(kBlockWide, 8);                                   \
+  } while (0)
+
+#define ROW_DISPATCH_MAX(nvec, LAUNCH)                         \
+  do {                                                         \
+    if ((nvec) <= kBlock) { LAUNCH(kBlock, 1); }               \
+    else if ((nvec) <= kBlock * 2) { LAUNCH(kBlock, 2); }      \
+    else if ((nvec) <= kBlock * 4) { LAUNCH(kBlock, 4); }      \
+    else if ((nvec) <= kBlockWide * 4) { LAUNCH(kBlockWide, 4); } \
+    else { LAUNCH(kBlockWide, 8); }                            \
+  } while (0)
+
 }
 
 void rmsnorm_fp8(torch::Tensor out, torch::Tensor out_scale, torch::Tensor x,
                  torch::Tensor weight, double eps) {
-  check_row_op(x, kBlock * 8 * kMaxVecPerThread);
+  check_row_op(x, kMaxH);
   const int H = x.size(-1);
   const int T = x.numel() / H;
-  hipLaunchKernelGGL((rmsnorm_fp8_kernel<false>), dim3(T), dim3(kBlock), 0,
-                     c10::hip::getCurrentHIPStream().stream(),
-                     (unsigned char*)out.data_ptr(),
-                     out_scale.data_ptr<float>(), (ushort*)x.data_ptr(),
-                     nullptr, (const ushort*)weight.data_ptr(), (float)eps, H);
+#define LAUNCH_ROW(THREADS, ITERS)                                          \
+  hipLaunchKernelGGL((rmsnorm_fp8_kernel<false, THREADS, ITERS>), dim3(T),  \
+                     dim3(THREADS), 0,                                      \
+                     c10::hip::getCurrentHIPStream().stream(),              \
+                     (unsigned char*)out.data_ptr(),                        \
+                     out_scale.data_ptr<float>(), (ushort*)x.data_ptr(),    \
+                     nullptr, (const ushort*)weight.data_ptr(), (float)eps, \
+                     H)
+  ROW_DISPATCH_NORM(H / 8, LAUNCH_ROW);
+#undef LAUNCH_ROW
   HIP_CHECK_KERNEL();
 }
 
 void fused_add_rmsnorm_fp8(torch::Tensor out, torch::Tensor out_scale,
                            torch::Tensor x, torch::Tensor residual,
                            torch::Tensor weight, double eps) {
-  check_row_op(x, kBlock * 8 * kMaxVecPerThread);
+  check_row_op(x, kMaxH);
   TORCH_CHECK(residual.is_contiguous());
   const int H = x.size(-1);
   const int T = x.numel() / H;
-  hipLaunchKernelGGL((rmsnorm_fp8_kernel<true>), dim3(T), dim3(kBlock), 0,
-                     c10::hip::getCurrentHIPStream().stream(),
-                     (unsigned char*)out.data_ptr(),
-                     out_scale.data_ptr<float>(), (ushort*)x.data_ptr(),
-                     (ushort*)residual.data_ptr(),
-                     (const ushort*)weight.data_ptr(), (float)eps, H);
+#define LAUNCH_ROW(THREADS, ITERS)                                          \
+  hipLaunchKernelGGL((rmsnorm_fp8_kernel<true, THREADS, ITERS>), dim3(T),   \
+                     dim3(THREADS), 0,                                      \
+                     c10::hip::getCurrentHIPStream().stream(),              \
+                     (unsigned char*)out.data_ptr(),                        \
+                     out_scale.data_ptr<float>(), (ushort*)x.data_ptr(),    \
+                     (ushort*)residual.data_ptr(),                          \
+                     (const ushort*)weight.data_ptr(), (float)eps, H)
+  ROW_DISPATCH_NORM(H / 8, LAUNCH_ROW);
+#undef LAUNCH_ROW
   HIP_CHECK_KERNEL();
 }
 
 void silu_and_mul_fp8(torch::Tensor out, torch::Tensor out_scale,
                       torch::Tensor x) {
-  check_row_op(x, 2 * kBlock * 8 * kMaxVecPerThread);
+  check_row_op(x, 2 * kMaxH);
   const int I = x.size(1) / 2;
-  TORCH_CHECK(I % 8 == 0 && I <= kBlock * 8 * kMaxVecPerThread);
+  TORCH_CHECK(I % 8 == 0 && I <= kMaxH);
   const int T = x.size(0);
   if (T == 0) return;
-  hipLaunchKernelGGL(silu_and_mul_fp8_kernel, dim3(T), dim3(kBlock), 0,
-                     c10::hip::getCurrentHIPStream().stream(),
-                     (unsigned char*)out.data_ptr(),
-                     out_scale.data_ptr<float>(),
-                     (const ushort*)x.data_ptr(), I);
+#define LAUNCH_ROW(THREADS, ITERS)                                          \
+  hipLaunchKernelGGL((silu_and_mul_fp8_kernel<THREADS, ITERS>), dim3(T),    \
+                     dim3(THREADS), 0,                                      \
+                     c10::hip::getCurrentHIPStream().stream(),              \
+                     (unsigned char*)out.data_ptr(),                        \
+                     out_scale.data_ptr<float>(),                           \
+                     (const ushort*)x.data_ptr(), I)
+  ROW_DISPATCH_MAX(I / 8, LAUNCH_ROW);
+#undef LAUNCH_ROW
   HIP_CHECK_KERNEL();
 }
 
 void quant_fp8(torch::Tensor out, torch::Tensor out_scale, torch::Tensor x) {
-  check_row_op(x, kBlock * 8 * kMaxVecPerThread);
+  check_row_op(x, kMaxH);
   const int H = x.size(-1);
   const int T = x.numel() / H;
   if (T == 0) return;
-  hipLaunchKernelGGL(quant_fp8_kernel, dim3(T), dim3(kBlock), 0,
-                     c10::hip::getCurrentHIPStream().stream(),
-                     (unsigned char*)out.data_ptr(),
-                     out_scale.data_ptr<float>(),
-                     (const ushort*)x.data_ptr(), H);
-  HIP_CHECK_KERNEL();
-}
+#define LAUNCH_ROW(THREADS, ITERS)                                          \
+  hipLaunchKernelGGL((quant_fp8_kernel<THREADS, ITERS>), dim3(T),           \
+                     dim3(THREADS), 0,                                      \
+                     c10::hip::getCurrentHIPStream().stream(),              \
+                     (unsigned char*)out.data_ptr(),                        \
+                     out_scale.data_ptr<float>(),                           \
+                     (const ushort*)x.data_ptr(), H)
+  ROW_DISPATCH_MAX(H / 8, LAUNCH_ROW);
+#undef LAUNCH_ROW
+  HIP_CHECK_KERNEL();
+}
diff --git a/kubeai_amd/csrc/rope.hip b/kubeai_amd/csrc/rope.hip
--- a/kubeai_amd/csrc/rope.hip
+++ b/kubeai_amd/csrc/rope.hip
@@ -31,8 +31,10 @@
     const float s = cs[half + i];
     const float x1 = bf16_to_f32(base[i]);
     const float x2 = bf16_to_f32(base[half + i]);
-    base[i] = f32_to_bf16(x1 * c - x2 * s);
-    base[half + i] = f32_to_bf16(x2 * c + x1 * s);
+    ushort o1, o2;
+    rope_rotate_pair(x1, x2, c, s, o1, o2);
+    base[i] = o1;
+    base[half + i] = o2;
   }
 }
 
diff --git a/kubeai_amd/csrc/rope_cache.hip b/kubeai_amd/csrc/rope_cache.hip
--- /dev/null
+++ b/kubeai_amd/csrc/rope_cache.hip
@@ -0,0 +1,137 @@
+#include <torch/extension.h>
+
+#include "common.h"
+
+namespace {
+
+DEV_INLINE void store_cache_elem(ushort* p, ushort bf) { *p = bf; }
+DEV_INLINE void store_cache_elem(unsigned char* p, ushort bf) {
+  *p = f32_to_e5m2(bf16_to_f32(bf));
+}
+
+template <typename CT>
+__global__ void rope_and_cache_kernel(
+    ushort* __restrict__ q,
+    ushort* __restrict__ k,
+    const ushort* __restrict__ v,
+    CT* __restrict__ k_cache,
+    CT* __restrict__ v_cache,
+    const int32_t* __restrict__ positions,
+    const float* __restrict__ cos_sin,
+    const int64_t* __restrict__ slot_mapping,
+    const int n_q, const int n_kv, const int hd, const int bs,
+    const int64_t n_tok, const int64_t q_stride, const int64_t k_stride,
+    const int64_t v_stride) {
+  const int n_heads = n_q + 2 * n_kv;
+  const int64_t flat = (int64_t)blockIdx.x * (blockDim.x / WAVE_SIZE) +
+                       threadIdx.x / WAVE_SIZE;
+  const int64_t tok = flat / n_heads;
+  if (tok >= n_tok) return;
+  const int head = (int)(flat % n_heads);
+  const int lane = threadIdx.x % WAVE_SIZE;
+
+  if (head >= n_q + n_kv) {
+    const int64_t slot = slot_mapping[tok];
+    if (slot < 0) return;
+    const int h = head - n_q - n_kv;
+    const ushort8* src =
+        reinterpret_cast<const ushort8*>(v + tok * v_stride + (int64_t)h * hd);
+    CT* dst = v_cache + (((slot / bs) * n_kv + h) * bs + slot % bs) * hd;
+    const int nvec = hd / 8;
+    for (int i = lane; i < nvec; i += WAVE_SIZE) {
+      const ushort8 vv = src[i];
+      if constexpr (sizeof(CT) == 2) {
+        reinterpret_cast<ushort8*>(dst)[i] = vv;
+      } else {
+        uint64_t vo = 0;
+#pragma unroll
+        for (int j = 0; j < 8; ++j)
+          vo |= (uint64_t)f32_to_e5m2(bf16_to_f32((ushort)vv[j])) << (8 * j);
+        reinterpret_cast<uint64_t*>(dst)[i] = vo;
+      }
+    }
+    return;
+  }
+
+  const int half = hd / 2;
+  const bool is_k = head >= n_q;
+  const int pos = positions[tok];
+  const float* cs = cos_sin + (int64_t)pos * hd;
+  ushort* base = is_k ? k + tok * k_stride + (int64_t)(head - n_q) * hd
+                      : q + tok * q_stride + (int64_t)head * hd;
+  CT* dst = nullptr;
+  if (is_k) {
+    const int64_t slot = slot_mapping[tok];
+    if (slot >= 0)
+      dst = k_cache +
+            (((slot / bs) * n_kv + (head - n_q)) * bs + slot % bs) * hd;
+  }
+  for (int i = lane; i < half; i += WAVE_SIZE) {
+    const float c = cs[i];
+    const float s = cs[half + i];
+    const float x1 = bf16_to_f32(base[i]);
+    const float x2 = bf16_to_f32(base[half + i]);
+    ushort o1, o2;
+    rope_rotate_pair(x1, x2, c, s, o1, o2);
+    base[i] = o1;
+    base[half + i] = o2;
+    if (dst != nullptr) {
+      store_cache_elem(dst + i, o1);
+      store_cache_elem(dst + half + i, o2);
+    }
+  }
+}
+
+}
+
+void rope_and_cache(torch::Tensor q, torch::Tensor k, torch::Tensor v,
+                    torch::Tensor positions, torch::Tensor cos_sin,
+                    torch::Tensor k_cache, torch::Tensor v_cache,
+                    torch::Tensor slot_mapping) {
+  TORCH_CHECK(q.dim() == 3 && k.dim() == 3 && v.dim() == 3);
+  TORCH_CHECK(q.stride(2) == 1 && q.stride(1) == q.size(2));
+  TORCH_CHECK(k.stride(2) == 1 && k.stride(1) == k.size(2));
+  TORCH_CHECK(v.stride(2) == 1 && v.stride(1) == v.size(2));
+  TORCH_CHECK(q.scalar_type() == torch::kBFloat16 &&
+              k.scalar_type() == torch::kBFloat16 &&
+              v.scalar_type() == torch::kBFloat16);
+  TORCH_CHECK(positions.scalar_type() == torch::kInt32);
+  TORCH_CHECK(cos_sin.scalar_type() == torch::kFloat32);
+  TORCH_CHECK(slot_mapping.scalar_type() == torch::kInt64);
+  TORCH_CHECK(k_cache.is_contiguous() && v_cache.is_contiguous());
+  TORCH_CHECK(k_cache.dim() == 4 && v_cache.sizes() == k_cache.sizes());
+  const bool fp8_cache = k_cache.scalar_type() == torch::kFloat8_e5m2;
+  TORCH_CHECK(fp8_cache || k_cache.scalar_type() == torch::kBFloat16);
+  TORCH_CHECK(v_cache.scalar_type() == k_cache.scalar_type());
+  const int T = q.size(0);
+  const int n_q = q.size(1), n_kv = k.size(1), hd = q.size(2);
+  TORCH_CHECK(hd == 128 || hd == 256,
+              "rope_and_cache supports head_dim 128 or 256");
+  TORCH_CHECK(k.size(0) == T && v.size(0) == T && k.size(2) == hd);
+  TORCH_CHECK(v.size(1) == n_kv && v.size(2) == hd);
+  TORCH_CHECK(cos_sin.size(1) == hd);
+  TORCH_CHECK(k_cache.size(1) == n_kv && k_cache.size(3) == hd);
+  TORCH_CHECK(positions.numel() >= T && slot_mapping.numel() >= T);
+  TORCH_CHECK(v.stride(0) % 8 == 0 && v.storage_offset() % 8 == 0);
+  const int bs = k_cache.size(2);
+  if (T == 0) return;
+  const int64_t total_waves = (int64_t)T * (n_q + 2 * n_kv);
+  const int waves_per_block = 4;
+  const int64_t blocks = (total_waves + waves_per_block - 1) / waves_per_block;
+#define LAUNCH_RC(CT)                                                        \
+  hipLaunchKernelGGL(                                                        \
+      (rope_and_cache_kernel<CT>), dim3((uint32_t)blocks),                   \
+      dim3(waves_per_block * WAVE_SIZE), 0,                                  \
+      c10::hip::getCurrentHIPStream().stream(), (ushort*)q.data_ptr(),       \
+      (ushort*)k.data_ptr(), (const ushort*)v.data_ptr(),                    \
+      (CT*)k_cache.data_ptr(), (CT*)v_cache.data_ptr(),                      \
+      positions.data_ptr<int32_t>(), cos_sin.data_ptr<float>(),              \
+      slot_mapping.data_ptr<int64_t>(), n_q, n_kv, hd, bs, (int64_t)T,       \
+      q.stride(0), k.stride(0), v.stride(0))
+  if (fp8_cache)
+    LAUNCH_RC(unsigned char);
+  else
+    LAUNCH_RC(ushort);
+#undef LAUNCH_RC
+  HIP_CHECK_KERNEL();
+}
diff --git a/kubeai_amd/models/llama.py b/kubeai_amd/models/llama.py
--- a/kubeai_amd/models/llama.py
+++ b/kubeai_amd/models/llama.py
@@ -90,17 +90,31 @@
         if self.qk_norm:
             q = _rms_head(q, self.q_norm, self.norm_eps)
             k = _rms_head(k, self.k_norm, self.norm_eps)
-            v = v.contiguous()
         if isinstance(cos_sin, tuple):
             cos_sin = cos_sin[0] if self.is_global else cos_sin[1]
-        q, k = ops.rope(q, k, fb.positions, cos_sin)
         k_cache, v_cache = kv_cache
-        ops.reshape_and_cache(k, v, k_cache, v_cache, fb.slot_mapping)
+        q, k = ops.rope_and_cache(
+            q, k, v, fb.positions, cos_sin, k_cache, v_cache, fb.slot_mapping
+        )
 
         out = torch.empty(
             (T, self.n_q, self.hd), dtype=qkv.dtype, device=qkv.device
         )
         nd = fb.n_decode
+        if fp8_in and fb.n_prefill == 0 and nd == T and nd > 0:
+            _, a8, ascale = ops.paged_attention_decode(
+                q,
+                k_cache,
+                v_cache,
+                fb.decode_block_tables,
+                fb.decode_seq_lens,
+                self.scale,
+                out=out,
+                window=self.window,
+                softcap=self.softcap,
+                fp8_out=True,
+            )
+            return self.o_proj.forward_quantized(a8, ascale)
         if nd > 0:
             ops.paged_attention_decode(
                 q[:nd],
diff --git a/kubeai_amd/ops/__init__.py b/kubeai_amd/ops/__init__.py
--- a/kubeai_amd/ops/__init__.py
+++ b/kubeai_amd/ops/__init__.py
@@ -62,14 +62,38 @@
     ref.reshape_and_cache(k, v, k_cache, v_cache, slot_mapping)
 
 
+def rope_and_cache(q, k, v, positions, cos_sin, k_cache, v_cache, slot_mapping):
+    if q.is_cuda:
+        _require_ext()
+        _C.rope_and_cache(
+            q, k, v, positions, cos_sin, k_cache, v_cache, slot_mapping
+        )
+        return q, k
+    q, k = ref.rope(q, k, positions, cos_sin)
+    ref.reshape_and_cache(k, v, k_cache, v_cache, slot_mapping)
+    return q, k
+
+
 def paged_attention_decode(
     q, k_cache, v_cache, block_tables, seq_lens, scale: float, out=None,
-    window: int = 0, softcap: float = 0.0,
+    window: int = 0, softcap: float = 0.0, fp8_out: bool = False,
 ):
     if q.is_cuda:
         _require_ext()
         if out is None:
             out = torch.empty(q.shape, dtype=q.dtype, device=q.device)
+        if fp8_out:
+            B = q.shape[0]
+            o8 = torch.empty(
+                (B, q.shape[1] * q.shape[2]), dtype=torch.float8_e4m3fn,
+                device=q.device,
+            )
+            oscale = torch.empty(B, dtype=torch.float32, device=q.device)
+            _C.paged_attention_decode_fp8(
+                out, o8, oscale, q, k_cache, v_cache, block_tables, seq_lens,
+                scale, window, softcap
+            )
+            return out, o8, oscale
         _C.paged_attention_decode(
             out, q, k_cache, v_cache, block_tables, seq_lens, scale, window,
             softcap
@@ -81,7 +105,10 @@
     )
     if out is not None:
         out.copy_(res)
-        return out
+        res = out
+    if fp8_out:
+        o8, oscale = ref.quant_fp8(res.reshape(res.shape[0], -1))
+        return res, o8, oscale
     return res
 
 
diff --git a/kubeai_amd/parallel/tp.py b/kubeai_amd/parallel/tp.py
--- a/kubeai_amd/parallel/tp.py
+++ b/kubeai_amd/parallel/tp.py
@@ -127,13 +127,21 @@
         q = q.unflatten(-1, (self.n_q, self.hd))
         k = k.unflatten(-1, (self.n_kv, self.hd))
         v = v.unflatten(-1, (self.n_kv, self.hd))
-        q, k = ops.rope(q, k, fb.positions, cos_sin)
         k_cache, v_cache = kv_cache
-        ops.reshape_and_cache(k, v, k_cache, v_cache, fb.slot_mapping)
+        q, k = ops.rope_and_cache(
+            q, k, v, fb.positions, cos_sin, k_cache, v_cache, fb.slot_mapping
+        )
         out = torch.empty(
             (T, self.n_q, self.hd), dtype=qkv.dtype, device=qkv.device
         )
         nd = fb.n_decode
+        if fp8_in and fb.n_prefill == 0 and nd == T and nd > 0:
+            _, a8, ascale = ops.paged_attention_decode(
+                q, k_cache, v_cache,
+                fb.decode_block_tables, fb.decode_seq_lens, self.scale,
+                out=out, window=getattr(self, "window", 0), fp8_out=True,
+            )
+            return self.o_proj.forward_quantized(a8, ascale)
         if nd > 0:
             ops.paged_attention_decode(
                 q[:nd], k_cache, v_cache,
```
